# Bhasha-Open/Akshar

Hardware: NVIDIA B200
Metric: utf8_input_GBps_batch_encode (higher is better)
Workload: dtype u8

## Files before the change

akshar_b200/csrc/ak_abi_encode.inc:

```
extern "C" {

struct AkTokOut {
    void* ids;
    int64_t id_cap;
    int ids_u16;
    void* splits;
    int splits_i32;
};
static int ak_run_tok(akshar_ctx* ctx, AkCall& C, const AkBatch& B, int64_t max_bytes, int kind, const AkTokOut& O) {
    int rc;
    const AkTokWs W = ak_tok_ws(max_bytes, B.n_rows);
    char* base = C.ws + C.L.scratch;
    const size_t avail = C.ws_bytes - C.L.scratch;
    const size_t surplus = avail > W.total ? ((avail - W.total) / 4) & ~(size_t)255 : 0;
    const size_t pool_ints = W.pool_ints + surplus / 4, longpool_ints = W.longpool_ints + surplus / 4;
    char* longpool = base + W.longpool + surplus;
    char* sl = base + W.slots + 2 * surplus;
    const size_t left = avail - (W.slots + 2 * surplus) - 4096;
    const double per_wt = (double)left / ((double)W.n_wt * (AKT_SLOT_BYTES + 0.001));
    int cap = AKT_CAP_MIN, shift = 8;
    while (cap < AKT_CAP_MAX && (double)(2 * cap) <= per_wt) { cap *= 2; ++shift; }
    const size_t n_slots = (size_t)W.n_wt * (size_t)cap;
    AkSlots S;
    S.ev = (AkEvent*)sl;
    S.count = (uint32_t*)(base + W.count);
    S.cap = cap;
    S.shift = shift;
    unsigned long long* resolved = (unsigned long long*)(sl + ak_align(n_slots * 8));
    uint32_t* aux = (uint32_t*)(sl + 2 * ak_align(n_slots * 8));
    int32_t* wt_ids = (int32_t*)(base + W.wt_ids);
    int64_t* wt_base = (int64_t*)(base + W.wt_base);
    unsigned long long* wt_seg = (unsigned long long*)(base + W.wt_seg);
    float* wt_segx = (float*)(base + W.wt_segx);
    const size_t nscan = ak_align(((size_t)W.n_wt / AKS_TILE + 2) * 8);
    unsigned long long* scan_state0 = (unsigned long long*)(base + W.scan_state);
    unsigned long long* scan_state1 = (unsigned long long*)(base + W.scan_state + nscan);
    AkcTable& tc = ctx->tok_cache[kind];
    if (!ctx->wc_hold || tc.reset) {
        const unsigned long long limit = (1ull << tc.work.bits) / 4;
        ak_cache_guard_kernel<<<ctx->sm_count * 4, 256, 0, C.stream>>>(tc.work.e, tc.image, tc.bytes / 8, tc.work.inserted, limit, tc.reset ? 1 : 0);
        if ((rc = ak_after_launch(ctx, "tok-cache-guard"))) return rc;
        ak_cache_guard_reset_kernel<<<1, 1, 0, C.stream>>>(tc.work.inserted, limit, tc.reset ? 1 : 0);
        if ((rc = ak_after_launch(ctx, "tok-cache-guard-reset"))) return rc;
        tc.reset = false;
    }
    AK_CUDA(ctx, cudaMemsetAsync(base + W.row_flag, 0, ak_align((size_t)B.n_rows + 1), C.stream));
    AK_CUDA(ctx, cudaMemsetAsync(scan_state0, 0, 2 * nscan, C.stream));
    int* tickets = (int*)C.ws;
    unsigned int* any_flag = (unsigned int*)(C.ws + 144);
    unsigned long long* pool_used = (unsigned long long*)(C.ws + 152);
    const int64_t base0 = B.text_begin - (int64_t)(((uintptr_t)B.text + (uintptr_t)B.text_begin) & 15u);
    const int64_t span = (B.dyn_end ? max_bytes : B.text_end) - base0;
    const int64_t n_wt_ub = (span + AKT_WARP_BYTES) / AKT_WARP_BYTES;
    AkWordsArgs A;
    A.B = B;
    A.T = ctx->T;
    A.bpe = ctx->bpe_d;
    A.base0 = base0;
    A.wrow = (const int64_t*)(base + W.wrow);
    A.S = S;
    A.row_flag = (uint8_t*)(base + W.row_flag);
    A.any_flag = any_flag;
    A.row_ev = (uint32_t*)(base + W.row_ev);
    long long* n_wt_dev = (long long*)(C.ws + 136);
    A.n_wt_out = n_wt_dev;
    const int entries = (int)(n_wt_ub * 2 + 3);
    ak_warp_rows_kernel<<<(entries + 255) / 256, 256, 0, C.stream>>>(B, base0, entries, (int64_t*)(base + W.wrow));
    if ((rc = ak_after_launch(ctx, "tok-warp-rows"))) return rc;
    if (kind == 1) {
        ak_long_rows_kernel<<<ctx->sm_count * 4, 256, 0, C.stream>>>(B, AKT_LONG_ROW, A.row_flag, any_flag);
        if ((rc = ak_after_launch(ctx, "tok-long-rows"))) return rc;
    }
    {
        AkTimed tm(ctx, AKSHAR_TIMER_WORDS, C.stream);
        const int g = ak_grid(ctx, ctx->occ_words[kind], (int)((n_wt_ub + AKW_THREADS / 32 - 1) / (AKW_THREADS / 32)));
        if (kind == 0) ak_words_kernel<0><<<g, AKW_THREADS, 0, C.stream>>>(A);
        else ak_words_kernel<1><<<g, AKW_THREADS, 0, C.stream>>>(A);
    }
    if ((rc = ak_after_launch(ctx, "tok-words"))) return rc;
    AkLookupCtx X;
    X.M.kind = kind;
    X.M.bpe = ctx->bpe_d;
    X.M.uni = ctx->uni_d;
    X.M.cache = tc.work;
    X.M.pool.base = (int32_t*)longpool;
    X.M.pool.used = (unsigned long long*)(C.ws + 128);
    X.M.pool.cap = longpool_ints;
    X.M.T = ctx->T;
    X.text = nullptr;
    X.off = nullptr;
    X.n_rows = 0;
    X.tb = X.te = 0;
    X.result = nullptr;
    X.ids = O.ids;
    X.id_cap = O.id_cap;
    X.ids_u16 = O.ids_u16;
    X.splits = O.splits;
    X.splits_i32 = O.splits_i32;
    X.row_flag = A.row_flag;
    X.row_fix = (unsigned long long*)(base + W.row_fix);
    X.pool = (int32_t*)(base + W.pool);
    X.pool_used = pool_used;
    X.pool_cap = pool_ints;
    X.any_fix = 0;
    AkRowFixArgs R;
    R.B = B;
    R.X.M = X.M;
    R.X.text = nullptr;
    R.X.off = nullptr;
    R.X.n_rows = 0;
    R.X.result = nullptr;
    R.X.ev = S.ev;
    R.X.n_events = 0;
    R.X.row_ev = A.row_ev;
    R.X.row_fix = (unsigned long long*)(base + W.row_fix);
    R.X.pool = X.pool;
    R.X.pool_used = pool_used;
    R.X.pool_cap = pool_ints;
    R.base0 = base0;
    R.cap = cap;
    R.row_flag = A.row_flag;
    R.any_flag = any_flag;
    ak_rowfix_kernel<<<ctx->sm_count * 8, 128, 0, C.stream>>>(R);
    if ((rc = ak_after_launch(ctx, "tok-rowfix"))) return rc;
    const int warp_ctas = (int)((n_wt_ub + AKL_THREADS / 32 - 1) / (AKL_THREADS / 32));
    const int scan_tiles = (int)(n_wt_ub / AKS_TILE + 1);
    unsigned int* status_word = (unsigned int*)&B.result[2];
    AkResolveArgs Rs;
    Rs.B = B;
    Rs.X = X;
    Rs.base0 = base0;
    Rs.S = S;
    Rs.resolved = resolved;
    Rs.aux = aux;
    Rs.wt_ids = wt_ids;
    Rs.wt_seg = wt_seg;
    Rs.any_flag = any_flag;
    {
        AkTimed tm(ctx, kind == 0 ? AKSHAR_TIMER_BPE_ENCODE : AKSHAR_TIMER_UNIGRAM, C.stream);
        const int g = ak_grid(ctx, ctx->occ_resolve[kind], warp_ctas);
        if (kind == 0) ak_resolve_kernel<0><<<g, AKR_THREADS, 0, C.stream>>>(Rs);
        else ak_resolve_kernel<1><<<g, AKR_THREADS, 0, C.stream>>>(Rs);
    }
    if ((rc = ak_after_launch(ctx, "tok-resolve"))) return rc;
    if (kind == 1) {
        ak_scan_seg_kernel<<<ak_grid(ctx, 4, scan_tiles), AKS_THREADS, 0, C.stream>>>(wt_seg, n_wt_dev, wt_segx, tickets + 4, scan_state1, status_word);
        if ((rc = ak_after_launch(ctx, "tok-scan-seg"))) return rc;
        AkCheckArgs Ck;
        Ck.B = B;
        Ck.X = X;
        Ck.base0 = base0;
        Ck.S = S;
        Ck.resolved = resolved;
        Ck.aux = aux;
        Ck.wt_seg_before = wt_segx;
        Ck.wt_ids = wt_ids;
        Ck.any_flag = any_flag;
        ak_unicheck_kernel<<<ak_grid(ctx, ctx->occ_check, warp_ctas), AKL_THREADS, 0, C.stream>>>(Ck);
        if ((rc = ak_after_launch(ctx, "tok-check"))) return rc;
    }
    ak_scan_counts_kernel<<<ak_grid(ctx, 4, scan_tiles), AKS_THREADS, 0, C.stream>>>(wt_ids, 0, n_wt_dev, 1, wt_base, B.totals, tickets + 5, scan_state0,
                                                                                    status_word);
    if ((rc = ak_after_launch(ctx, "tok-scan-ids"))) return rc;
    AkEmitArgs E;
    E.B = B;
    E.X = X;
    E.base0 = base0;
    E.S = S;
    E.resolved = resolved;
    E.wt_base = wt_base;
    E.any_flag = any_flag;
    {
        AkTimed tm(ctx, AKSHAR_TIMER_EMIT, C.stream);
        if (O.ids_u16) ak_emit_kernel<uint16_t><<<ak_grid(ctx, ctx->occ_emit, warp_ctas), AKL_THREADS, 0, C.stream>>>(E);
        else ak_emit_kernel<int32_t><<<ak_grid(ctx, ctx->occ_emit, warp_ctas), AKL_THREADS, 0, C.stream>>>(E);
    }
    return ak_after_launch(ctx, "tok-emit");
}

static int ak_run_bpe(akshar_ctx* ctx, AkCall& C, const AkBatch& B, int64_t max_bytes, const AkTokOut& O) {
    return ak_run_tok(ctx, C, B, max_bytes, 0, O);
}

static int ak_run_unigram(akshar_ctx* ctx, AkCall& C, const AkBatch& B, int64_t max_bytes, const AkTokOut& O, int mode) {
    if (mode == AKSHAR_MODE_TILES && ctx->uni_fast) return ak_run_tok(ctx, C, B, max_bytes, 1, O);
    if (O.ids_u16 || O.splits_i32) {
        ctx->err = "compact outputs need AKSHAR_MODE_TILES and a model of the shape scripts/train_spm.py writes";
        return AKSHAR_E_ARG;
    }
    int32_t* d_ids = (int32_t*)O.ids;
    int64_t* d_id_splits = (int64_t*)O.splits;
    const int64_t id_capacity = O.id_cap;
    const size_t tiles = (size_t)ak_tiles_of(max_bytes, B.n_rows);
    AkUniArgs A;
    A.B = B;
    A.B.mode = AKSHAR_MODE_ROWS;
    A.B.n_tiles = (int)((B.n_rows + AK_ROWS_BLOCK - 1) / AK_ROWS_BLOCK);
    A.B.ticket = (int*)C.ws + 1;
    A.B.state0 = C.B.state0 + 1 * tiles;
    A.U = ctx->uni_d;
    A.back = (uint32_t*)(C.ws + C.L.scratch);
    A.back_cap = (int64_t)((C.ws_bytes - C.L.scratch) / 4);
    A.ids = d_ids;
    A.id_cap = id_capacity;
    A.id_splits = d_id_splits;
    {
        AkTimed tm(ctx, AKSHAR_TIMER_UNIGRAM, C.stream);
        ak_unigram_kernel<<<ak_grid(ctx, ctx->occ_uni, A.B.n_tiles), AK_ROWS_BLOCK, 0, C.stream>>>(A);
    }
    return ak_after_launch(ctx, "unigram");
}

int akshar_encode_bpe_batch(akshar_ctx* ctx, const uint8_t* d_text, const int64_t* d_row_offsets, int64_t n_rows,
                            int64_t text_begin, int64_t text_end, int mode, int32_t* d_ids, int64_t id_capacity,
                            int64_t* d_id_splits, int64_t* d_result, void* d_workspace, size_t workspace_bytes,
                            void* stream) {
    AkDeviceGuard device_guard(ctx ? ctx->device : 0);
    AkCall C;
    int rc = ak_begin(ctx, d_text, d_row_offsets, n_rows, text_begin, text_end, mode, 0, d_result, d_workspace, workspace_bytes,
                      stream, C);
    if (rc) return rc;
    if (!ctx->has_bpe) {
        ctx->err = "no BPE model loaded";
        return AKSHAR_E_NOMODEL;
    }
    if (!d_id_splits || id_capacity < 0 || (!d_ids && id_capacity > 0)) {
        ctx->err = "bad argument";
        return AKSHAR_E_ARG;
    }
    if (n_rows == 0) return ak_empty_rows(ctx, d_id_splits, nullptr, C.stream);
    const AkTokOut O = {d_ids, id_capacity, 0, d_id_splits, 0};
    return ak_run_bpe(ctx, C, C.B, text_end - text_begin, O);
}

int akshar_encode_unigram_batch(akshar_ctx* ctx, const uint8_t* d_text, const int64_t* d_row_offsets, int64_t n_rows,
                                int64_t text_begin, int64_t text_end, int mode, int32_t* d_ids, int64_t id_capacity,
                                int64_t* d_id_splits, int64_t* d_result, void* d_workspace, size_t workspace_bytes,
                                void* stream) {
    AkDeviceGuard device_guard(ctx ? ctx->device : 0);
    AkCall C;
    if (mode != AKSHAR_MODE_TILES && mode != AKSHAR_MODE_ROWS) return AKSHAR_E_ARG;
    int rc = ak_begin(ctx, d_text, d_row_offsets, n_rows, text_begin, text_end, AKSHAR_MODE_ROWS, AK_ROWS_BLOCK, d_result,
                      d_workspace, workspace_bytes, stream, C);
    if (rc) return rc;
    if (!ctx->has_uni) {
        ctx->err = "no Unigram model loaded";
        return AKSHAR_E_NOMODEL;
    }
    if (!d_id_splits || id_capacity < 0 || (!d_ids && id_capacity > 0)) {
        ctx->err = "bad argument";
        return AKSHAR_E_ARG;
    }
    if (n_rows == 0) return ak_empty_rows(ctx, d_id_splits, nullptr, C.stream);
    const AkTokOut O = {d_ids, id_capacity, 0, d_id_splits, 0};
    return ak_run_unigram(ctx, C, C.B, text_end - text_begin, O, mode);
}

int akshar_tokenizer_encode_batch(akshar_ctx* ctx, const uint8_t* d_text, const int64_t* d_row_offsets, int64_t n_rows,
                                  int64_t text_begin, int64_t text_end, uint32_t norm_flags, int kind, int mode,
                                  uint8_t* d_norm_text, int64_t norm_capacity, int64_t* d_norm_row_offsets, int32_t* d_ids,
                                  int64_t id_capacity, int64_t* d_id_splits, int64_t* d_result, void* d_workspace,
                                  size_t workspace_bytes, void* stream) {
    return akshar_tokenizer_encode_batch_ex(ctx, d_text, d_row_offsets, n_rows, text_begin, text_end, norm_flags, kind, mode,
                                            d_norm_text, norm_capacity, d_norm_row_offsets, d_ids, id_capacity, d_id_splits, 0u,
                                            d_result, d_workspace, workspace_bytes, stream);
}

int akshar_tokenizer_encode_batch_ex(akshar_ctx* ctx, const uint8_t* d_text, const int64_t* d_row_offsets, int64_t n_rows,
                                     int64_t text_begin, int64_t text_end, uint32_t norm_flags, int kind, int mode,
                                     uint8_t* d_norm_text, int64_t norm_capacity, int64_t* d_norm_row_offsets, void* d_ids,
                                     int64_t id_capacity, void* d_id_splits, uint32_t out_flags, int64_t* d_result,
                                     void* d_workspace, size_t workspace_bytes, void* stream) {
    AkDeviceGuard device_guard(ctx ? ctx->device : 0);
    if (!ctx) return AKSHAR_E_ARG;
    if (norm_capacity < 0 || !d_norm_row_offsets || (!d_norm_text && norm_capacity > 0) || (norm_flags & ~15u) ||
        (kind != 0 && kind != 1) || !d_id_splits || id_capacity < 0 || (!d_ids && id_capacity > 0) || (out_flags & ~3u)) {
        ctx->err = "bad argument";
        return AKSHAR_E_ARG;
    }
    if ((out_flags & AKSHAR_OUT_IDS_U16) && akshar_vocab_size(ctx, kind) > 65536) {
        ctx->err = "uint16 ids need a vocabulary of at most 65536 entries";
        return AKSHAR_E_ARG;
    }
    if (kind == 0 ? !ctx->has_bpe : !ctx->has_uni) {
        ctx->err = "no model loaded for this encoder";
        return AKSHAR_E_NOMODEL;
    }
    const int64_t n_bytes = text_end - text_begin;
    const int64_t max_bytes = n_bytes > norm_capacity ? n_bytes : norm_capacity;
    if (workspace_bytes < ak_ws_layout(max_bytes, n_rows).total) {
        ctx->err = "workspace too small: need " + std::to_string(ak_ws_layout(max_bytes, n_rows).total) + " bytes";
        return AKSHAR_E_WORKSPACE;
    }
    AkCall C;
    int rc = ak_begin(ctx, d_text, d_row_offsets, n_rows, text_begin, text_end, mode, 0, d_result, d_workspace, workspace_bytes,
                      stream, C);
    if (rc) return rc;
    C.L = ak_ws_layout(max_bytes, n_rows);
    const size_t tiles = (size_t)ak_tiles_of(max_bytes, n_rows);
    AK_CUDA(ctx, cudaMemsetAsync(C.ws, 0, 256 + ak_align(4 * tiles * 8), C.stream));
    C.B.state0 = (unsigned long long*)(C.ws + C.L.state);
    C.B.state1 = C.B.state0 + tiles;
    if (n_rows == 0) {
        AK_CUDA(ctx, cudaMemsetAsync(d_id_splits, 0, sizeof(int64_t), C.stream));
        return ak_empty_rows(ctx, d_norm_row_offsets, nullptr, C.stream);
    }
    AkBatch B1 = C.B;
    B1.totals = d_result + 1;
    if ((rc = ak_run_normalize(ctx, C, B1, norm_flags, d_norm_text, norm_capacity, d_norm_row_offsets))) return rc;
    AkBatch B2 = C.B;
    B2.text = d_norm_text;
    B2.off = d_norm_row_offsets;
    B2.text_begin = 0;
    B2.text_end = 0;
    B2.dyn_end = d_result + 1;
    if (mode != AKSHAR_MODE_TILES) B2.n_tiles = (int)((n_rows + AK_BLOCK - 1) / AK_BLOCK);
    const AkTokOut O = {d_ids, id_capacity, (out_flags & AKSHAR_OUT_IDS_U16) ? 1 : 0, d_id_splits, (out_flags & AKSHAR_OUT_SPLITS_I32) ? 1 : 0};
    if (kind == 0) return ak_run_bpe(ctx, C, B2, max_bytes, O);
    return ak_run_unigram(ctx, C, B2, max_bytes, O, mode);
}

}
```

akshar_b200/csrc/ak_abi_text.inc:

```
static int ak_run_normalize(akshar_ctx* ctx, AkCall& C, const AkBatch& B, uint32_t flags, uint8_t* out, int64_t out_cap,
                            int64_t* out_off) {
    const bool raw_fast = flags == AK_NORM_ROMAN;
    if ((flags == (AK_NORM_ROMAN | AK_NORM_CLEAN) || raw_fast) && B.mode == AKSHAR_MODE_TILES && !B.dyn_end) {
        AkFastNormArgs F;
        F.flags = flags;
        F.B = B;
        F.T = ctx->T;
        F.out = out;
        F.out_cap = out_cap;
        F.out_off = out_off;
        F.base0 = B.text_begin - (int64_t)(((uintptr_t)B.text + (uintptr_t)B.text_begin) & 15u);
        F.B.n_tiles = (int)((B.text_end - F.base0 + AKF_TILE) / AKF_TILE);
        int64_t* tile_row = (int64_t*)(C.ws + C.L.tile_row);
        F.tile_row = tile_row;
        const int entries = F.B.n_tiles * AKF_WARPS + 1;
        ak_warp_rows_kernel<<<(entries + 255) / 256, 256, 0, C.stream>>>(B, F.base0, entries, tile_row);
        int rc = ak_after_launch(ctx, "warp-rows");
        if (rc) return rc;
        AkNfWork W;
        const size_t nt = (size_t)F.B.n_tiles;
        char* wp = C.ws + C.L.scratch;
        W.info = (uint32_t*)wp;                         wp += ak_align(nt * AK_BLOCK * 4);
        W.tile_total = (int32_t*)wp;                    wp += ak_align(nt * AKF_WARPS * 4);
        W.tile_base = (int64_t*)wp;                     wp += ak_align((nt * AKF_WARPS + 1) * 8);
        W.slow = (AkSlowEntry*)wp;
        W.n_slow = (unsigned int*)(C.ws + 72);
        W.slow_cap = (unsigned int)(nt * AK_BLOCK / 16 + 1024);
        {
            AkTimed tm(ctx, AKSHAR_TIMER_NORMALIZE_CLASSIFY, C.stream);
            ak_nf3_classify_kernel<<<ak_grid(ctx, ctx->occ_nf3, F.B.n_tiles), AKN3_THREADS, 0, C.stream>>>(F, W);
        }
        if ((rc = ak_after_launch(ctx, "normalize-classify"))) return rc;
        AkNfSlowArgs S;
        S.B = B;
        S.T = ctx->T;
        S.W = W;
        S.tile_row = tile_row;
        S.out = out;
        S.out_cap = out_cap;
        S.out_off = out_off;
        S.write = 0;
        S.flags = flags;
        const int slow_grid = ctx->sm_count * AKN_SLOW_MINB;
        ak_nf_slow_kernel<<<slow_grid, 128, 0, C.stream>>>(S);
        if ((rc = ak_after_launch(ctx, "normalize-slow-count"))) return rc;
        const long long n_wtiles = (long long)F.B.n_tiles * AKF_WARPS;
        ak_scan_counts_kernel<<<ak_grid(ctx, 4, (int)(n_wtiles / AKS_TILE + 1)), AKS_THREADS, 0, C.stream>>>(
            W.tile_total, n_wtiles, nullptr, 1, W.tile_base, B.totals, (int*)C.ws + 6, C.B.state1,
            (unsigned int*)&B.result[2]);
        if ((rc = ak_after_launch(ctx, "normalize-scan"))) return rc;
        {
            AkTimed tm(ctx, AKSHAR_TIMER_NORMALIZE_WRITE, C.stream);
            ak_nf_write_kernel<<<ak_grid(ctx, ctx->occ_nf_write, F.B.n_tiles), AK_BLOCK, 0, C.stream>>>(F, W);
        }
        if ((rc = ak_after_launch(ctx, "normalize-write"))) return rc;
        S.write = 1;
        ak_nf_slow_kernel<<<slow_grid, 128, 0, C.stream>>>(S);
        return ak_after_launch(ctx, "normalize-slow-write");
    }
    AkNormArgs A;
    A.B = B;
    A.T = ctx->T;
    A.flags = flags;
    A.out = out;
    A.out_cap = out_cap;
    A.out_off = out_off;
    ak_normalize_kernel<<<ak_grid(ctx, ctx->occ_norm, A.B.n_tiles), AK_BLOCK, 0, C.stream>>>(A);
    return ak_after_launch(ctx, "normalize");
}

int akshar_normalize_batch(akshar_ctx* ctx, const uint8_t* d_text, const int64_t* d_row_offsets, int64_t n_rows,
                           int64_t text_begin, int64_t text_end, uint32_t flags, int mode, uint8_t* d_out_text,
                           int64_t out_capacity, int64_t* d_out_row_offsets, int64_t* d_result, void* d_workspace,
                           size_t workspace_bytes, void* stream) {
    AkDeviceGuard device_guard(ctx ? ctx->device : 0);
    AkCall C;
    int rc = ak_begin(ctx, d_text, d_row_offsets, n_rows, text_begin, text_end, mode, 0, d_result, d_workspace, workspace_bytes,
                      stream, C);
    if (rc) return rc;
    if (!d_out_row_offsets || out_capacity < 0 || (!d_out_text && out_capacity > 0) || (flags & ~15u)) {
        ctx->err = "bad argument";
        return AKSHAR_E_ARG;
    }
    if (n_rows == 0) return ak_empty_rows(ctx, d_out_row_offsets, nullptr, C.stream);
    return ak_run_normalize(ctx, C, C.B, flags, d_out_text, out_capacity, d_out_row_offsets);
}

static int ak_run_seg_mask(akshar_ctx* ctx, AkCall& C, const AkBatch& B, int64_t max_bytes, uint32_t flags, uint32_t* cmask,
                           uint32_t* rmask, uint32_t* tags, int64_t n_words) {
    int rc;
    AkSegMaskArgs M;
    M.B = B;
    M.T = ctx->T;
    M.flags = flags;
    M.shift = (int)(((uintptr_t)B.text + (uintptr_t)B.text_begin) & 15u);
    M.base0 = B.text_begin - M.shift;
    M.cmask = cmask;
    M.rmask = rmask;
    M.t0 = tags;
    M.t1 = tags ? tags + n_words : nullptr;
    M.n_words = n_words;
    const int64_t n_wt = (B.text_begin + max_bytes - M.base0 + AKN3_WARP_BYTES) / AKN3_WARP_BYTES;
    int64_t* wrow = (int64_t*)(C.ws + C.L.scratch);
    M.wrow = wrow;
    const int entries = (int)(n_wt * 2 + 3);
    ak_warp_rows_kernel<<<(entries + 255) / 256, 256, 0, C.stream>>>(B, M.base0, entries, wrow);
    if ((rc = ak_after_launch(ctx, "segment-warp-rows"))) return rc;
    {
        AkTimed tm(ctx, AKSHAR_TIMER_SEGMENT, C.stream);
        ak_seg_mask_kernel<<<ak_grid(ctx, 8, (int)((n_wt + AKSM_THREADS / 32 - 1) / (AKSM_THREADS / 32))), AKSM_THREADS, 0, C.stream>>>(M);
    }
    return ak_after_launch(ctx, "segment-mask");
}

int akshar_segment_batch(akshar_ctx* ctx, const uint8_t* d_text, const int64_t* d_row_offsets, int64_t n_rows,
                         int64_t text_begin, int64_t text_end, uint32_t flags, int mode, int32_t* d_cluster_ends,
                         int64_t cluster_capacity, int64_t* d_cluster_splits, int32_t* d_run_ends, uint8_t* d_run_tags,
                         int64_t run_capacity, int64_t* d_run_splits, int64_t* d_result, void* d_workspace,
                         size_t workspace_bytes, void* stream) {
    AkDeviceGuard device_guard(ctx ? ctx->device : 0);
    AkCall C;
    int rc = ak_begin(ctx, d_text, d_row_offsets, n_rows, text_begin, text_end, mode, 0, d_result, d_workspace, workspace_bytes,
                      stream, C);
    if (rc) return rc;
    const bool want_c = (flags & AKSHAR_SEG_CLUSTERS) != 0, want_r = (flags & AKSHAR_SEG_RUNS) != 0;
    if (flags & AKSHAR_SEG_MASK) {
        const int64_t n_words = (text_end - text_begin + 32) / 32;
        if ((flags & ~15u) || (!want_c && !want_r) || ((flags & AKSHAR_SEG_MATRAS) && !want_c) || mode != AKSHAR_MODE_TILES ||
            (want_c && (!d_cluster_ends || cluster_capacity < n_words)) ||
            (want_r && (!d_run_ends || !d_run_tags || run_capacity < n_words))) {
            ctx->err = "bad argument (AKSHAR_SEG_MASK: tile mode, capacities in 32-bit words >= (bytes + 32) / 32)";
            return AKSHAR_E_ARG;
        }
        return ak_run_seg_mask(ctx, C, C.B, text_end - text_begin, flags & 7u, (uint32_t*)d_cluster_ends, (uint32_t*)d_run_ends,
                               (uint32_t*)d_run_tags, n_words);
    }
    if ((flags & ~7u) || (!want_c && !want_r) || ((flags & AKSHAR_SEG_MATRAS) && !want_c) ||
        (want_c && (!d_cluster_splits || cluster_capacity < 0 || (!d_cluster_ends && cluster_capacity > 0))) ||
        (want_r && (!d_run_splits || run_capacity < 0 || ((!d_run_ends || !d_run_tags) && run_capacity > 0)))) {
        ctx->err = "bad argument";
        return AKSHAR_E_ARG;
    }
    if (n_rows == 0) return ak_empty_rows(ctx, want_c ? d_cluster_splits : nullptr, want_r ? d_run_splits : nullptr, C.stream);
    AkSegArgs A;
    A.B = C.B;
    A.T = ctx->T;
    A.flags = flags;
    A.o.cluster_ends = d_cluster_ends;
    A.o.cluster_splits = d_cluster_splits;
    A.o.run_ends = d_run_ends;
    A.o.run_tags = d_run_tags;
    A.o.run_splits = d_run_splits;
    A.o.cbase = A.o.rbase = 0;
    A.o.ccap = want_c ? cluster_capacity : 0;
    A.o.rcap = want_r ? run_capacity : 0;
    if (mode == AKSHAR_MODE_TILES) {
        AkSegOffArgs F;
        F.B = C.B;
        F.T = ctx->T;
        F.flags = flags;
        F.base0 = text_begin - (int64_t)(((uintptr_t)d_text + (uintptr_t)text_begin) & 15u);
        const int64_t n_wt = (text_end - F.base0 + AKN3_WARP_BYTES) / AKN3_WARP_BYTES;
        char* wp = C.ws + C.L.scratch;
        int64_t* wrow = (int64_t*)wp;       wp += ak_align(((size_t)n_wt * 2 + 3) * 8);
        F.c_count = (int32_t*)wp;           wp += ak_align((size_t)n_wt * 4);
        F.r_count = (int32_t*)wp;           wp += ak_align((size_t)n_wt * 4);
        int64_t* c_base = (int64_t*)wp;     wp += ak_align((size_t)n_wt * 8);
        int64_t* r_base = (int64_t*)wp;
        F.wrow = wrow;
        F.c_base = c_base;
        F.r_base = r_base;
        F.o = A.o;
        const int entries = (int)(n_wt * 2 + 3);
        ak_warp_rows_kernel<<<(entries + 255) / 256, 256, 0, C.stream>>>(C.B, F.base0, entries, wrow);
        if ((rc = ak_after_launch(ctx, "segment-warp-rows"))) return rc;
        const int grid = ak_grid(ctx, 8, (int)((n_wt + AKSO_THREADS / 32 - 1) / (AKSO_THREADS / 32)));
        ak_seg_off_kernel<false><<<grid, AKSO_THREADS, 0, C.stream>>>(F);
        if ((rc = ak_after_launch(ctx, "segment-count"))) return rc;
        const int sgrid = ak_grid(ctx, 4, (int)(n_wt / AKS_TILE + 1));
        if (want_c) {
            ak_scan_counts_kernel<<<sgrid, AKS_THREADS, 0, C.stream>>>(F.c_count, (long long)n_wt, nullptr, 1, c_base, d_result,
                                                                       (int*)C.ws + 5, C.B.state0, (unsigned int*)&d_result[2]);
            if ((rc = ak_after_launch(ctx, "segment-scan"))) return rc;
        }
        if (want_r) {
            ak_scan_counts_kernel<<<sgrid, AKS_THREADS, 0, C.stream>>>(F.r_count, (long long)n_wt, nullptr, 1, r_base, d_result + 1,
                                                                       (int*)C.ws + 6, C.B.state1, (unsigned int*)&d_result[2]);
            if ((rc = ak_after_launch(ctx, "segment-scan"))) return rc;
        }
        {
            AkTimed tm(ctx, AKSHAR_TIMER_SEGMENT, C.stream);
            ak_seg_off_kernel<true><<<grid, AKSO_THREADS, 0, C.stream>>>(F);
        }
        return ak_after_launch(ctx, "segment-emit");
    }
    ak_segment_kernel<<<ak_grid(ctx, ctx->occ_seg, A.B.n_tiles), AK_BLOCK, 0, C.stream>>>(A);
    return ak_after_launch(ctx, "segment");
}

int akshar_word_tokenize_batch(akshar_ctx* ctx, const uint8_t* d_text, const int64_t* d_row_offsets, int64_t n_rows,
                               int64_t text_begin, int64_t text_end, int rule, int32_t* d_word_begin, int32_t* d_word_end,
                               int64_t word_capacity, int64_t* d_word_splits, uint8_t* d_row_flags, int64_t* d_result,
                               void* d_workspace, size_t workspace_bytes, void* stream) {
    AkDeviceGuard device_guard(ctx ? ctx->device : 0);
    AkCall C;
    int rc = ak_begin(ctx, d_text, d_row_offsets, n_rows, text_begin, text_end, AKSHAR_MODE_TILES, 0, d_result, d_workspace,
                      workspace_bytes, stream, C);
    if (rc) return rc;
    if ((rule != AKSHAR_WORDS_HINDI && rule != AKSHAR_WORDS_SPLIT) || !d_word_splits || word_capacity < 0 ||
        ((!d_word_begin || !d_word_end) && word_capacity > 0)) {
        ctx->err = "bad argument";
        return AKSHAR_E_ARG;
    }
    if (n_rows == 0) return ak_empty_rows(ctx, d_word_splits, nullptr, C.stream);
    if (d_row_flags) AK_CUDA(ctx, cudaMemsetAsync(d_row_flags, 0, (size_t)n_rows, C.stream));
    AkWtArgs A;
    A.B = C.B;
    A.base0 = text_begin - (int64_t)(((uintptr_t)d_text + (uintptr_t)text_begin) & 15u);
    const int64_t n_wt = (text_end - A.base0 + AKT_WARP_BYTES) / AKT_WARP_BYTES;
    char* wp = C.ws + C.L.scratch;
    int64_t* wrow = (int64_t*)wp;       wp += ak_align(((size_t)n_wt * 2 + 3) * 8);
    A.count = (int32_t*)wp;             wp += ak_align((size_t)n_wt * 4);
    int64_t* wt_base = (int64_t*)wp;
    A.wrow = wrow;
    A.base = wt_base;
    A.mode = rule == AKSHAR_WORDS_HINDI ? AKW_MODE_HINDI : AKW_MODE_SPLIT;
    A.begin = d_word_begin;
    A.end = d_word_end;
    A.cap = word_capacity;
    A.splits = d_word_splits;
    A.row_flags = d_row_flags;
    const int entries = (int)(n_wt * 2 + 3);
    ak_warp_rows_kernel<<<(entries + 255) / 256, 256, 0, C.stream>>>(C.B, A.base0, entries, wrow);
    if ((rc = ak_after_launch(ctx, "words-warp-rows"))) return rc;
    const int grid = ak_grid(ctx, 8, (int)((n_wt + AKWT_THREADS / 32 - 1) / (AKWT_THREADS / 32)));
    ak_wtok_kernel<false><<<grid, AKWT_THREADS, 0, C.stream>>>(A);
    if ((rc = ak_after_launch(ctx, "words-count"))) return rc;
    ak_scan_counts_kernel<<<ak_grid(ctx, 4, (int)(n_wt / AKS_TILE + 1)), AKS_THREADS, 0, C.stream>>>(
        A.count, (long long)n_wt, nullptr, 1, wt_base, d_result, (int*)C.ws + 5, C.B.state0, (unsigned int*)&d_result[2]);
    if ((rc = ak_after_launch(ctx, "words-scan"))) return rc;
    {
        AkTimed tm(ctx, AKSHAR_TIMER_WORDTOK, C.stream);
        ak_wtok_kernel<true><<<grid, AKWT_THREADS, 0, C.stream>>>(A);
    }
    return ak_after_launch(ctx, "words-emit");
}
```

akshar_b200/csrc/ak_common.cuh:

```cuda
#pragma once
#define AK_BLOCK 256
#define AK_SPAN 32
#define AK_TILE (AK_BLOCK * AK_SPAN)
#define AK_LOOKBACK_LIMIT 4096
#define AK_ROWS_BLOCK 128
#define AKF_WARPS (AK_BLOCK / 32)
#define AKF_TILE (AKF_WARPS * AKF_WARP_BYTES)

static_assert((int)AK_ST_OVERFLOW == (int)AKSHAR_ST_OVERFLOW && (int)AK_ST_NFC_SEGMENT == (int)AKSHAR_ST_NFC_SEGMENT &&
              (int)AK_ST_PATHOLOGICAL == (int)AKSHAR_ST_PATHOLOGICAL && (int)AK_ST_ALPHABET == (int)AKSHAR_ST_ALPHABET &&
              (int)AK_ST_SPIN == (int)AKSHAR_ST_SPIN && (int)AK_ST_WORD == (int)AKSHAR_ST_WORD &&
              (int)AK_ST_INTERNAL == (int)AKSHAR_ST_INTERNAL && (int)AK_ST_BAD_ID == (int)AKSHAR_ST_BAD_ID, "status bits out of sync");
static_assert(AK_NORM_ROMAN == AKSHAR_NORM_ROMAN && AK_NORM_CLEAN == AKSHAR_NORM_CLEAN && AK_NORM_FILTER == AKSHAR_NORM_FILTER &&
              AK_NORM_COLLAPSE == AKSHAR_NORM_COLLAPSE && AK_NORM_NO_NFC == AKSHAR_NORM_NO_NFC, "flags out of sync");
static_assert(AK_SEG_CLUSTERS == AKSHAR_SEG_CLUSTERS && AK_SEG_MATRAS == AKSHAR_SEG_MATRAS &&
              AK_SEG_RUNS == AKSHAR_SEG_RUNS, "flags out of sync");

struct AkBatch {
    const uint8_t* text;
    const int64_t* off;
    int64_t n_rows, text_begin, text_end;
    int mode;
    int n_tiles;
    int* ticket;
    unsigned long long* state0;
    unsigned long long* state1;
    int64_t* result;
    int64_t* totals;
    const unsigned int* run_if;
    const int64_t* dyn_end;
};

__device__ __forceinline__ bool ak_batch_begin(AkBatch& B) {
    if (B.run_if && *B.run_if == 0) return false;
    if (B.dyn_end) {
        if (B.result[2] & (AK_ST_OVERFLOW | AK_ST_PATHOLOGICAL | AK_ST_NFC_SEGMENT | AK_ST_SPIN)) return false;
        B.text_end = B.text_begin + *B.dyn_end;
        if (B.mode == AKSHAR_MODE_TILES) B.n_tiles = (int)((B.text_end - B.text_begin + AK_TILE) / AK_TILE);
    }
    return true;
}

struct AkSpan {
    int64_t s, e, r_lo, r_hi, limit;
};

__device__ __forceinline__ void ak_raise(int64_t* result, uint32_t bits) {
    if (bits) atomicOr((unsigned long long*)&result[2], (unsigned long long)bits);
}

__device__ __forceinline__ AkSpan ak_span_of(const AkBatch& B, int tile, int64_t* sh) {
    AkSpan sp;
    if (B.mode == AKSHAR_MODE_TILES) {
        const int64_t t0 = B.text_begin + (int64_t)tile * AK_TILE;
        int64_t t1 = t0 + AK_TILE;
        if (t1 > B.text_end + 1) t1 = B.text_end + 1;
        if (threadIdx.x == 0) {
            int64_t lo = ak_row_lower_bound(B.off, 0, B.n_rows, t0);
            sh[0] = lo > 0 ? lo - 1 : 0;
            sh[1] = ak_row_lower_bound(B.off, lo, B.n_rows, t1);
        }
        __syncthreads();
        sp.r_lo = sh[0];
        sp.r_hi = sh[1];
        sp.s = t0 + (int64_t)threadIdx.x * AK_SPAN;
        sp.e = sp.s + AK_SPAN;
        if (sp.e > t1) sp.e = t1;
        if (sp.s > sp.e) sp.s = sp.e;
        sp.limit = AK_LOOKBACK_LIMIT;
    } else {
        const int64_t r = (int64_t)tile * AK_BLOCK + threadIdx.x;
        sp.r_lo = 0;
        sp.r_hi = B.n_rows;
        sp.limit = 0;
        if (r < B.n_rows) {
            sp.s = B.off[r];
            sp.e = (r == B.n_rows - 1) ? B.text_end + 1 : B.off[r + 1];
        } else {
            sp.s = sp.e = 0;
        }
    }
    return sp;
}

__device__ __forceinline__ int ak_next_tile(int* ticket, int* sh) {
    __syncthreads();
    if (threadIdx.x == 0) *sh = atomicAdd(ticket, 1);
    __syncthreads();
    return *sh;
}



__global__ void ak_warp_rows_kernel(AkBatch B, int64_t base0, int n_entries, int64_t* wrow) {
    if (!ak_batch_begin(B)) return;
    const int k = blockIdx.x * blockDim.x + threadIdx.x;
    if (k >= n_entries) return;
    const int64_t pos = base0 + (int64_t)k * AKF_WARP_BYTES;
    int64_t r = ak_row_lower_bound(B.off, 0, B.n_rows, pos);
    if (B.off[r] < pos) r = B.n_rows + 1;
    wrow[k] = r;
}


#define AKN3_THREADS 128
#define AKN3_WARP_BYTES 960

__device__ __forceinline__ uint32_t akn3_lane_rows(const int64_t* off, int64_t n_rows, int64_t r_w0, int64_t ws, int lane) {
    uint32_t rows = 0;
    const int64_t lo = ws - 32, hi = ws + AKN3_WARP_BYTES + 32;
    for (int64_t r = r_w0;; r += 32) {
        const int64_t mr = r + lane;
        const int64_t p = mr <= n_rows ? off[mr] : hi;
        const unsigned m = __ballot_sync(0xFFFFFFFFu, p < hi);
        const int cnt = __popc(m);
        for (int j = 0; j < cnt; ++j) {
            const int rel = (int)(__shfl_sync(0xFFFFFFFFu, p, j) - lo);
            if ((rel >> 5) == lane) rows |= 1u << (rel & 31);
        }
        if (cnt < 32) break;
    }
    for (int64_t r = r_w0 - 1;; r -= 32) {
        const int64_t mr = r - lane;
        const int64_t p = mr >= 0 ? off[mr] : lo - 1;
        const unsigned m = __ballot_sync(0xFFFFFFFFu, p >= lo);
        const int cnt = __popc(m);
        for (int j = 0; j < cnt; ++j) {
            const int rel = (int)(__shfl_sync(0xFFFFFFFFu, p, j) - lo);
            if ((rel >> 5) == lane) rows |= 1u << (rel & 31);
        }
        if (cnt < 32) break;
    }
    return rows;
}

__device__ __forceinline__ uint32_t akn3_lane_rows2(const int64_t* off, int64_t n_rows, int64_t r_w0, int64_t ws, int lane,
                                                    int64_t& first_row, int& nrows) {
    uint32_t rows = 0;
    int64_t first = 0x7FFFFFFFFFFFFFFFll;
    int cntl = 0;
    const int64_t lo = ws - 32, hi = ws + AKN3_WARP_BYTES + 32;
    for (int64_t r = r_w0;; r += 32) {
        const int64_t mr = r + lane;
        const int64_t p = mr <= n_rows ? off[mr] : hi;
        const unsigned m = __ballot_sync(0xFFFFFFFFu, p < hi);
        const int cnt = __popc(m);
        for (int j = 0; j < cnt; ++j) {
            const int rel = (int)(__shfl_sync(0xFFFFFFFFu, p, j) - lo);
            if ((rel >> 5) == lane) {
                rows |= 1u << (rel & 31);
                ++cntl;
                if (r + j < first) first = r + j;
            }
        }
        if (cnt < 32) break;
    }
    for (int64_t r = r_w0 - 1;; r -= 32) {
        const int64_t mr = r - lane;
        const int64_t p = mr >= 0 ? off[mr] : lo - 1;
        const unsigned m = __ballot_sync(0xFFFFFFFFu, p >= lo);
        const int cnt = __popc(m);
        for (int j = 0; j < cnt; ++j) {
            const int rel = (int)(__shfl_sync(0xFFFFFFFFu, p, j) - lo);
            if ((rel >> 5) == lane) {
                rows |= 1u << (rel & 31);
                ++cntl;
                if (r - j < first) first = r - j;
            }
        }
        if (cnt < 32) break;
    }
    first_row = first;
    nrows = cntl;
    return rows;
}

__device__ __forceinline__ void akn3_load_edge(const uint8_t* text, int64_t cs, int lo, int hi, uint32_t* x) {
#pragma unroll
    for (int w = 0; w < 8; ++w) {
        uint32_t v = 0;
#pragma unroll
        for (int b = 0; b < 4; ++b) {
            const int i = 4 * w + b;
            if (i >= lo && i < hi) v |= (uint32_t)text[cs + i] << (8 * b);
        }
        x[w] = v;
    }
}
```

akshar_b200/csrc/ak_kernels.cu:

```cuda
#include <cuda_runtime.h>
#include <math.h>
#include <stdio.h>
#include <stdlib.h>
#include <string.h>

#include <exception>
#include <new>
#include <string>
#include <vector>

#include "../../include/akshar_b200.h"
#include "ak_models.h"
#include "ak_scan.cuh"
#include "ak_subword.cuh"
#include "ak_fast.cuh"
#include "ak_norm3.cuh"
#include "ak_seg3.cuh"
#include "ak_bpe3.cuh"
#include "ak_tok.cuh"
#include "ak_tok_host.h"
#include "ak_decode_host.h"
#include "unicode_tables.inc"


#include "ak_common.cuh"
#include "ak_norm_kernels.cuh"
#include "ak_seg_kernels.cuh"
#include "ak_sub_kernels.cuh"
#include "ak_tok_kernels.cuh"
#include "ak_wtok_kernels.cuh"
#include "ak_decode_kernels.cuh"
#include "ak_feat_kernels.cuh"
#include "ak_lines_kernels.cuh"

struct AkcTable {
    AkWordCache work{};
    unsigned long long* image = nullptr;
    size_t bytes = 0;
    bool reset = false;
};

struct akshar_ctx {
    int device = 0;
    int sm_count = 148;
    AkTables T{};
    std::vector<void*> allocs;
    std::string err;
    int64_t launches = 0;
    bool has_bpe = false, has_uni = false;
    AkBpeHost bpe_h;
    AkBpeDev bpe_d{};
    AkUniHost uni_h;
    AkUniDev uni_d{};
    std::vector<void*> bpe_allocs, uni_allocs;
    AkcTable tok_cache[2];
    AkDecTable dec[2][2] = {};
    bool uni_fast = false;
    int occ_words[2] = {0, 0}, occ_resolve[2] = {0, 0}, occ_check = 0, occ_emit = 0;
    bool timing = false;
    bool wc_hold = false;
    cudaEvent_t tev[AKSHAR_TIMER_COUNT][2] = {};
    bool tev_valid[AKSHAR_TIMER_COUNT] = {};
    int occ_norm = 0, occ_seg = 0, occ_uni = 0, occ_sig = 0, occ_nf_write = 0, occ_nf3 = 0;
};

struct AkDeviceGuard {
    int prev = -1;
    bool switched = false;
    explicit AkDeviceGuard(int dev) {
        if (cudaGetDevice(&prev) == cudaSuccess && prev != dev) switched = cudaSetDevice(dev) == cudaSuccess;
    }
    ~AkDeviceGuard() {
        if (switched) cudaSetDevice(prev);
    }
};

#define AK_CUDA(ctx, call)                                                                         \
    do {                                                                                           \
        cudaError_t e_ = (call);                                                                   \
        if (e_ != cudaSuccess) {                                                                   \
            (ctx)->err = std::string(#call) + ": " + cudaGetErrorString(e_);                       \
            return AKSHAR_E_CUDA;                                                                  \
        }                                                                                          \
    } while (0)

template <class V>
static int ak_upload(akshar_ctx* ctx, std::vector<void*>& owner, const V* src, size_t n, const V** dst) {
    void* d = nullptr;
    size_t bytes = (n ? n : 1) * sizeof(V);
    AK_CUDA(ctx, cudaMalloc(&d, bytes));
    owner.push_back(d);
    if (n) AK_CUDA(ctx, cudaMemcpy(d, src, n * sizeof(V), cudaMemcpyHostToDevice));
    *dst = (const V*)d;
    return 0;
}

extern "C" {

int akshar_version(void) { return 100; }

const char* akshar_status_str(int code) {
    switch (code) {
        case AKSHAR_OK: return "ok";
        case AKSHAR_E_ARG: return "bad argument";
        case AKSHAR_E_CUDA: return "CUDA error";
        case AKSHAR_E_MODEL: return "model could not be parsed or uses an unsupported configuration";
        case AKSHAR_E_NOMODEL: return "no model loaded for this encoder";
        case AKSHAR_E_WORKSPACE: return "workspace too small";
        default: return "unknown";
    }
}

int akshar_ctx_create(int device, akshar_ctx** out) {
    if (!out) return AKSHAR_E_ARG;
    *out = nullptr;
    akshar_ctx* ctx = new (std::nothrow) akshar_ctx();
    if (!ctx) return AKSHAR_E_ARG;
    ctx->device = device;
    *out = ctx;
    AkDeviceGuard device_guard(device);
    AK_CUDA(ctx, cudaSetDevice(device));
    cudaDeviceProp prop;
    AK_CUDA(ctx, cudaGetDeviceProperties(&prop, device));
    if (prop.major < 10) {
        ctx->err = "akshar_b200 is built for sm_100a (B200); device is sm_" + std::to_string(prop.major * 10 + prop.minor);
        return AKSHAR_E_CUDA;
    }
    ctx->sm_count = prop.multiProcessorCount;
    int rc;
#define UP(field, arr, n, type) \
    if ((rc = ak_upload<type>(ctx, ctx->allocs, (const type*)(arr), (size_t)(n), (const type**)&ctx->T.field))) return rc;
    UP(page_index, ak_tbl_page_index, AK_N_PAGES, uint16_t)
    UP(leaves, ak_tbl_leaves, AK_N_LEAF_PAGES * 256, uint32_t)
    UP(decomp_keys, ak_tbl_decomp_keys, AK_N_DECOMP, uint32_t)
    UP(decomp_off, ak_tbl_decomp_off, AK_N_DECOMP + 1, uint16_t)
    UP(decomp_data, ak_tbl_decomp_data, AK_N_DECOMP_DATA, uint32_t)
    UP(pair_keys, ak_tbl_pair_keys, AK_N_PAIRS, unsigned long long)
    UP(pair_vals, ak_tbl_pair_vals, AK_N_PAIRS, uint32_t)
    UP(ll_keys, ak_tbl_latin_lower_keys, AK_N_LATIN_LOWER, uint32_t)
    UP(ll_vals, ak_tbl_latin_lower_vals, AK_N_LATIN_LOWER, uint32_t)
    UP(fl_keys, ak_tbl_full_lower_keys, AK_N_FULL_LOWER, uint32_t)
    UP(fl_vals, ak_tbl_full_lower_vals, AK_N_FULL_LOWER, uint32_t)
    UP(kmap_keys, ak_tbl_kmap_keys, AK_N_KMAP, uint32_t)
    UP(kmap_off, ak_tbl_kmap_off, AK_N_KMAP + 1, uint16_t)
    UP(kmap_data, ak_tbl_kmap_data, AK_N_KMAP_DATA, uint32_t)
    UP(hf_unknown, ak_tbl_hf_unknown, AK_N_HF_UNKNOWN, uint32_t)
#undef UP
    ctx->T.n_decomp = AK_N_DECOMP;
    ctx->T.n_pairs = AK_N_PAIRS;
    ctx->T.n_ll = AK_N_LATIN_LOWER;
    ctx->T.n_fl = AK_N_FULL_LOWER;
    ctx->T.n_kmap = AK_N_KMAP;
    ctx->T.n_hf_unknown = AK_N_HF_UNKNOWN;
    AK_CUDA(ctx, cudaOccupancyMaxActiveBlocksPerMultiprocessor(&ctx->occ_norm, ak_normalize_kernel, AK_BLOCK, 0));
    AK_CUDA(ctx, cudaOccupancyMaxActiveBlocksPerMultiprocessor(&ctx->occ_nf_write, ak_nf_write_kernel, AK_BLOCK, 0));
    AK_CUDA(ctx, cudaOccupancyMaxActiveBlocksPerMultiprocessor(&ctx->occ_nf3, ak_nf3_classify_kernel, AKN3_THREADS, 0));
    AK_CUDA(ctx, cudaOccupancyMaxActiveBlocksPerMultiprocessor(&ctx->occ_seg, ak_segment_kernel, AK_BLOCK, 0));
    AK_CUDA(ctx, cudaOccupancyMaxActiveBlocksPerMultiprocessor(&ctx->occ_uni, ak_unigram_kernel, AK_ROWS_BLOCK, 0));
    AK_CUDA(ctx, cudaOccupancyMaxActiveBlocksPerMultiprocessor(&ctx->occ_sig, ak_signature_kernel, AK_ROWS_BLOCK, 0));
    AK_CUDA(ctx, cudaOccupancyMaxActiveBlocksPerMultiprocessor(&ctx->occ_words[0], ak_words_kernel<0>, AKW_THREADS, 0));
    AK_CUDA(ctx, cudaOccupancyMaxActiveBlocksPerMultiprocessor(&ctx->occ_words[1], ak_words_kernel<1>, AKW_THREADS, 0));
    AK_CUDA(ctx, cudaOccupancyMaxActiveBlocksPerMultiprocessor(&ctx->occ_resolve[0], ak_resolve_kernel<0>, AKR_THREADS, 0));
    AK_CUDA(ctx, cudaOccupancyMaxActiveBlocksPerMultiprocessor(&ctx->occ_resolve[1], ak_resolve_kernel<1>, AKR_THREADS, 0));
    AK_CUDA(ctx, cudaOccupancyMaxActiveBlocksPerMultiprocessor(&ctx->occ_check, ak_unicheck_kernel, AKL_THREADS, 0));
    AK_CUDA(ctx, cudaOccupancyMaxActiveBlocksPerMultiprocessor(&ctx->occ_emit, ak_emit_kernel<int32_t>, AKL_THREADS, 0));
    return AKSHAR_OK;
}

static void ak_free_list(std::vector<void*>& v) {
    for (void* p : v) cudaFree(p);
    v.clear();
}

void akshar_ctx_destroy(akshar_ctx* ctx) {
    if (!ctx) return;
    AkDeviceGuard device_guard(ctx->device);
    ak_free_list(ctx->allocs);
    ak_free_list(ctx->bpe_allocs);
    ak_free_list(ctx->uni_allocs);
    for (int i = 0; i < AKSHAR_TIMER_COUNT; ++i)
        for (int k = 0; k < 2; ++k)
            if (ctx->tev[i][k]) cudaEventDestroy(ctx->tev[i][k]);
    delete ctx;
}

const char* akshar_last_error(akshar_ctx* ctx) { return ctx ? ctx->err.c_str() : "null context"; }

int akshar_word_cache_hold(akshar_ctx* ctx, int hold) {
    if (!ctx) return AKSHAR_E_ARG;
    if (hold < 0) {
        ctx->tok_cache[0].reset = ctx->tok_cache[1].reset = true;
        return AKSHAR_OK;
    }
    ctx->wc_hold = hold != 0;
    return AKSHAR_OK;
}

int akshar_timing_enable(akshar_ctx* ctx, int enable) {
    AkDeviceGuard device_guard(ctx ? ctx->device : 0);
    if (!ctx) return AKSHAR_E_ARG;
    AK_CUDA(ctx, cudaSetDevice(ctx->device));
    if (enable)
        for (int i = 0; i < AKSHAR_TIMER_COUNT; ++i)
            for (int k = 0; k < 2; ++k)
                if (!ctx->tev[i][k]) AK_CUDA(ctx, cudaEventCreate(&ctx->tev[i][k]));
    ctx->timing = enable != 0;
    for (int i = 0; i < AKSHAR_TIMER_COUNT; ++i) ctx->tev_valid[i] = false;
    return AKSHAR_OK;
}

int akshar_timing_read(akshar_ctx* ctx, int timer, float* ms) {
    if (!ctx || !ms || timer < 0 || timer >= AKSHAR_TIMER_COUNT) return AKSHAR_E_ARG;
    if (!ctx->tev_valid[timer]) return AKSHAR_E_ARG;
    AK_CUDA(ctx, cudaEventSynchronize(ctx->tev[timer][1]));
    AK_CUDA(ctx, cudaEventElapsedTime(ms, ctx->tev[timer][0], ctx->tev[timer][1]));
    return AKSHAR_OK;
}

int64_t akshar_launch_count(akshar_ctx* ctx) { return ctx ? ctx->launches : 0; }

static inline size_t ak_align(size_t x) { return (x + 255) & ~(size_t)255; }
static inline int64_t ak_tiles_of(int64_t n_bytes, int64_t n_rows) {
    int64_t a = (n_bytes + n_bytes / 8 + 1024 + 32 + AKF_TILE - 1) / AKF_TILE;
    int64_t b = (n_rows + AK_ROWS_BLOCK - 1) / AK_ROWS_BLOCK;
    return (a > b ? a : b) + 1;
}
struct AkTokWs {
    size_t wrow, count, wt_ids, wt_base, wt_seg, wt_segx, scan_state, row_flag, row_ev, row_fix, pool, longpool, slots, total;
    size_t pool_ints, longpool_ints;
    int64_t n_wt;
};
#define AKT_CAP_MIN 256
#define AKT_CAP_MAX 2048
#define AKT_SLOT_BYTES 20
static AkTokWs ak_tok_ws(int64_t n_bytes, int64_t n_rows) {
    AkTokWs W;
    W.n_wt = n_bytes / AKT_WARP_BYTES + 3;
    size_t at = 0;
    W.wrow = at;       at += ak_align(((size_t)W.n_wt * 2 + 4) * 8);
    W.count = at;      at += ak_align((size_t)W.n_wt * 4);
    W.wt_ids = at;     at += ak_align((size_t)W.n_wt * 4);
    W.wt_base = at;    at += ak_align((size_t)W.n_wt * 8);
    W.wt_seg = at;     at += ak_align((size_t)W.n_wt * 8);
    W.wt_segx = at;    at += ak_align((size_t)W.n_wt * 4);
    W.scan_state = at; at += 2 * ak_align(((size_t)W.n_wt / AKS_TILE + 2) * 8);
    W.row_flag = at;   at += ak_align((size_t)n_rows + 1);
    W.row_ev = at;     at += ak_align(((size_t)n_rows + 2) * 4);
    W.row_fix = at;    at += ak_align(((size_t)n_rows + 1) * 8);
    W.pool_ints = (size_t)n_bytes / 4 + 65536;
    W.pool = at;       at += ak_align(W.pool_ints * 4);
    W.longpool_ints = (size_t)n_bytes / 8 + 65536;
    W.longpool = at;   at += ak_align(W.longpool_ints * 4);
    W.slots = at;
    at += (size_t)W.n_wt * AKT_CAP_MIN * (AKT_SLOT_BYTES + 1) + 8192;
    W.total = at;
    return W;
}

struct AkWsLayout {
    size_t control, state, tile_row, scratch, total;
};
static AkWsLayout ak_ws_layout(int64_t n_bytes, int64_t n_rows) {
    AkWsLayout L;
    size_t tiles = (size_t)ak_tiles_of(n_bytes, n_rows);
    L.control = 0;
    L.state = 256;
    L.tile_row = L.state + ak_align(4 * tiles * 8);
    size_t at = L.tile_row + ak_align(8 * (tiles * AKF_WARPS + 2));
    L.scratch = at;
    size_t m = 4 * (size_t)(n_bytes + 2 * n_rows + 2);
    const size_t nf = ak_align(tiles * AK_BLOCK * 4) + ak_align(tiles * AKF_WARPS * 4) + ak_align((tiles * AKF_WARPS + 1) * 8) +
                      ak_align((tiles * AK_BLOCK / 16 + 1024) * sizeof(AkSlowEntry));
    if (nf > m) m = nf;
    const size_t n_wt = (size_t)n_bytes / AKN3_WARP_BYTES + 3;
    const size_t sg = ak_align((2 * n_wt + 3) * 8) + 2 * ak_align(n_wt * 4) + 2 * ak_align(n_wt * 8);
    if (sg > m) m = sg;
    const size_t tok = ak_tok_ws(n_bytes, n_rows).total;
    if (tok > m) m = tok;
    L.total = at + ak_align(m);
    return L;
}

size_t akshar_workspace_bytes(int64_t n_bytes, int64_t n_rows) {
    if (n_bytes < 0 || n_rows < 0) return 0;
    return ak_ws_layout(n_bytes, n_rows).total;
}

struct AkCall {
    akshar_ctx* ctx;
    AkBatch B;
    AkWsLayout L;
    char* ws;
    size_t ws_bytes;
    cudaStream_t stream;
};

static int ak_begin(akshar_ctx* ctx, const uint8_t* d_text, const int64_t* d_row_offsets, int64_t n_rows, int64_t text_begin,
                    int64_t text_end, int mode, int rows_block, int64_t* d_result, void* d_workspace, size_t workspace_bytes,
                    void* stream, AkCall& C) {
    if (!ctx) return AKSHAR_E_ARG;
    if (!d_row_offsets || !d_result || n_rows < 0 || text_end < text_begin || (!d_text && text_end > text_begin) ||
        (mode != AKSHAR_MODE_TILES && mode != AKSHAR_MODE_ROWS)) {
        ctx->err = "bad argument";
        return AKSHAR_E_ARG;
    }
    const int64_t n_bytes = text_end - text_begin;
    if (n_bytes >= AKSHAR_MAX_CALL_BYTES || n_rows >= AKSHAR_MAX_CALL_ROWS) {
        ctx->err = "batch too large for one call: at most 4 GiB - 64 KiB of text and 2^29 - 1 rows; split it by row ranges";
        return AKSHAR_E_ARG;
    }
    C.ctx = ctx;
    C.L = ak_ws_layout(n_bytes, n_rows);
    if (!d_workspace || workspace_bytes < C.L.total) {
        ctx->err = "workspace too small: need " + std::to_string(C.L.total) + " bytes";
        return AKSHAR_E_WORKSPACE;
    }
    C.ws = (char*)d_workspace;
    C.ws_bytes = workspace_bytes;
    C.stream = (cudaStream_t)stream;
    AK_CUDA(ctx, cudaSetDevice(ctx->device));
    const size_t tiles = (size_t)ak_tiles_of(n_bytes, n_rows);
    AK_CUDA(ctx, cudaMemsetAsync(C.ws, 0, 256 + ak_align(4 * tiles * 8), C.stream));
    AK_CUDA(ctx, cudaMemsetAsync(d_result, 0, 4 * sizeof(int64_t), C.stream));
    AkBatch& B = C.B;
    B.text = d_text;
    B.off = d_row_offsets;
    B.n_rows = n_rows;
    B.text_begin = text_begin;
    B.text_end = text_end;
    B.mode = mode;
    if (rows_block > 0) B.n_tiles = (int)((n_rows + rows_block - 1) / rows_block);
    else if (mode == AKSHAR_MODE_TILES) B.n_tiles = (int)((n_bytes + 1 + AK_TILE - 1) / AK_TILE);
    else B.n_tiles = (int)((n_rows + AK_BLOCK - 1) / AK_BLOCK);
    B.ticket = (int*)C.ws;
    B.state0 = (unsigned long long*)(C.ws + C.L.state);
    B.state1 = B.state0 + tiles;
    B.result = d_result;
    B.totals = d_result;
    B.run_if = nullptr;
    B.dyn_end = nullptr;
    return AKSHAR_OK;
}

struct AkTimed {
    akshar_ctx* ctx;
    int slot;
    cudaStream_t s;
    AkTimed(akshar_ctx* c, int sl, cudaStream_t st) : ctx(c), slot(sl), s(st) {
        if (ctx->timing && ctx->tev[slot][0]) cudaEventRecord(ctx->tev[slot][0], s);
    }
    ~AkTimed() {
        if (ctx->timing && ctx->tev[slot][1]) { cudaEventRecord(ctx->tev[slot][1], s); ctx->tev_valid[slot] = true; }
    }
};

static int ak_grid(akshar_ctx* ctx, int occ, int n_tiles) {
    int g = ctx->sm_count * (occ > 0 ? occ : 1);
    return n_tiles < g ? (n_tiles > 0 ? n_tiles : 1) : g;
}

static int ak_after_launch(akshar_ctx* ctx, const char* what) {
    cudaError_t e = cudaGetLastError();
    static const bool debug_sync = getenv("AKSHAR_DEBUG_SYNC") != nullptr;
    if (e == cudaSuccess && debug_sync) {
        e = cudaDeviceSynchronize();
        if (e != cudaSuccess) fprintf(stderr, "akshar_b200: kernel '%s' failed: %s\n", what, cudaGetErrorString(e));
    }
    if (e != cudaSuccess) {
        ctx->err = std::string(what) + " launch: " + cudaGetErrorString(e);
        return AKSHAR_E_CUDA;
    }
    ctx->launches++;
    return AKSHAR_OK;
}

static int ak_empty_rows(akshar_ctx* ctx, int64_t* a, int64_t* b, cudaStream_t s) {
    if (a) AK_CUDA(ctx, cudaMemsetAsync(a, 0, sizeof(int64_t), s));
    if (b) AK_CUDA(ctx, cudaMemsetAsync(b, 0, sizeof(int64_t), s));
    return AKSHAR_OK;
}

#include "ak_abi_text.inc"

}

#include "ak_abi_aux.inc"
#include "ak_abi_models.inc"
#include "ak_abi_encode.inc"
```

akshar_b200/csrc/ak_norm_kernels.cuh:

```cuda
#pragma once
struct AkNormArgs {
    AkBatch B;
    AkTables T;
    uint32_t flags;
    uint8_t* out;
    int64_t out_cap;
    int64_t* out_off;
};

__global__ void __launch_bounds__(AK_BLOCK) ak_normalize_kernel(const AkNormArgs A) {
    __shared__ int ws[33];
    __shared__ int s_tile;
    __shared__ int64_t s_win[2];
    __shared__ long long s_base;
    AkBatch B = A.B;
    if (!ak_batch_begin(B)) return;
    for (;;) {
        const int tile = ak_next_tile(B.ticket, &s_tile);
        if (tile >= B.n_tiles) break;
        const AkSpan sp = ak_span_of(B, tile, s_win);
        uint32_t st = 0;
        int cnt = 0;
        if (sp.s < sp.e)
            cnt = (int)ak_norm_span(A.T, B.text, B.off, B.n_rows, sp.r_lo, sp.r_hi, sp.s, sp.e, A.flags, sp.limit, nullptr,
                                    nullptr, 0, st);
        int total;
        const int pre = ak_block_exscan<AK_BLOCK>(cnt, ws, total);
        if (threadIdx.x < 32) {
            long long b = ak_tile_prefix(B.state0, tile, total, (unsigned int*)&B.result[2], AK_ST_SPIN);
            if (threadIdx.x == 0) {
                s_base = b;
                if (tile == B.n_tiles - 1) B.totals[0] = b + total;
            }
        }
        __syncthreads();
        const int64_t obase = s_base + pre;
        if (sp.s < sp.e) {
            uint8_t* o = nullptr;
            if (obase + cnt <= A.out_cap) o = A.out + obase;
            else if (cnt > 0) st |= AK_ST_OVERFLOW;
            uint32_t st2 = 0;
            ak_norm_span(A.T, B.text, B.off, B.n_rows, sp.r_lo, sp.r_hi, sp.s, sp.e, A.flags, sp.limit, o, A.out_off, obase, st2);
        }
        ak_raise(B.result, st);
    }
}

struct AkFastNormArgs {
    AkBatch B;
    AkTables T;
    uint8_t* out;
    int64_t out_cap;
    int64_t* out_off;
    const int64_t* tile_row;
    int64_t base0;
    uint32_t flags;
};

__device__ __noinline__ void akf_load_edge(const uint8_t* text, int64_t cs, int lo, int hi, uint32_t* w) {
    w[0] = w[1] = w[2] = w[3] = 0;
#pragma unroll 1
    for (int i = lo; i < hi; ++i) w[i >> 2] |= (uint32_t)text[cs + i] << ((i & 3) * 8);
}

template <class CH>
__device__ __forceinline__ void akf_load_chunk(const uint8_t* text, int64_t cs, int64_t tb, int64_t te, CH& c) {
    int64_t lo = tb - cs, hi = te - cs;
    lo = lo < 0 ? 0 : (lo > 16 ? 16 : lo);
    hi = hi < 0 ? 0 : (hi > 16 ? 16 : hi);
    c.own = hi > lo ? (((1u << hi) - 1u) & ~((1u << lo) - 1u)) : 0u;
    if (c.own == 0xFFFFu) {
        const uint4 v = *reinterpret_cast<const uint4*>(text + cs);
        c.w[0] = v.x; c.w[1] = v.y; c.w[2] = v.z; c.w[3] = v.w;
    } else {
        uint32_t w[4];
        akf_load_edge(text, cs, (int)lo, (int)hi, w);
        c.w[0] = w[0]; c.w[1] = w[1]; c.w[2] = w[2]; c.w[3] = w[3];
    }
}


#define AK_SLOW_BYTES 72
struct AkSlowEntry {
    int64_t pos;
    int64_t out_base;
    int32_t cnt;
    int32_t tile;
    int32_t span;
    int32_t pad_;
    uint8_t bytes[AK_SLOW_BYTES];
};

struct AkNfWork {
    uint32_t* info;
    int32_t* tile_total;
    int64_t* tile_base;
    AkSlowEntry* slow;
    unsigned int* n_slow;
    unsigned int slow_cap;
};

template <class CH>
__device__ __forceinline__ void akf_load_lane(const AkBatch& B, int64_t cs, CH& c) {
    akf_load_chunk(B.text, cs, B.text_begin, B.text_end, c);
    uint32_t nx = __shfl_down_sync(0xFFFFFFFFu, c.w[0], 1);
    if ((threadIdx.x & 31) == 31) {
        nx = 0;
#pragma unroll
        for (int i = 0; i < 4; ++i) {
            const int64_t q = cs + 16 + i;
            if (q >= B.text_begin && q < B.text_end) nx |= (uint32_t)B.text[q] << (i * 8);
        }
    }
    c.w[4] = nx;
}


#ifndef AKN3_MINB
#define AKN3_MINB 8
#endif
__global__ void __launch_bounds__(AKN3_THREADS, AKN3_MINB) ak_nf3_classify_kernel(const AkFastNormArgs A, const AkNfWork W) {
    const AkBatch& B = A.B;
    const int tid = threadIdx.x, lane = tid & 31, warp = tid >> 5;
    const int64_t tb = B.text_begin, te = B.text_end;
    const bool raw = !(A.flags & AK_NORM_CLEAN);
    for (int tile = blockIdx.x; tile < B.n_tiles; tile += gridDim.x) {
        const int64_t tile_start = A.base0 + (int64_t)tile * AKF_TILE;
        const int64_t ws = tile_start + (int64_t)warp * AKN3_WARP_BYTES;
        const int64_t cs = ws + (int64_t)(lane - 1) * 32;
        AkN3Lane L;
        {
            uint32_t x[8];
            int64_t lo = tb - cs, hi = te - cs;
            lo = lo < 0 ? 0 : (lo > 32 ? 32 : lo);
            hi = hi < 0 ? 0 : (hi > 32 ? 32 : hi);
            if (lo == 0 && hi == 32) {
                const uint4 v0 = *reinterpret_cast<const uint4*>(B.text + cs);
                const uint4 v1 = *reinterpret_cast<const uint4*>(B.text + cs + 16);
                x[0] = v0.x; x[1] = v0.y; x[2] = v0.z; x[3] = v0.w;
                x[4] = v1.x; x[5] = v1.y; x[6] = v1.z; x[7] = v1.w;
                L.own = 0xFFFFFFFFu;
            } else {
                akn3_load_edge(B.text, cs, (int)lo, (int)hi, x);
                L.own = hi > lo ? ((hi == 32 ? 0xFFFFFFFFu : ((1u << hi) - 1u)) & ~((1u << lo) - 1u)) : 0u;
            }
            L.rows = akn3_lane_rows(B.off, B.n_rows, A.tile_row[(size_t)tile * AKF_WARPS + 2 * warp], ws, lane);
            akn3_phase1(x, L);
        }
        uint32_t up1p = __shfl_up_sync(0xFFFFFFFFu, L.up1, 1);
        uint32_t dn1n = __shfl_down_sync(0xFFFFFFFFu, L.dn1, 1);
        if (lane == 0) up1p = 0;
        if (lane == 31) dn1n = 0;
        akn3_phase2(L, up1p, dn1n, raw);
        uint32_t up2p = __shfl_up_sync(0xFFFFFFFFu, L.up2, 1);
        uint32_t dn2n = __shfl_down_sync(0xFFFFFFFFu, L.dn2, 1);
        if (lane == 0) up2p = AKN3_HALO_UP2;
        if (lane == 31) dn2n = 0;
        akn3_phase3(A.T, B.text, cs, te, L, up2p, dn2n, raw);
        {
            uint32_t rest = 0;
            if (L.ge) rest = akn3_gaps_local(B.text, cs, te, L);
            if (lane == 0) {
                akn3_gaps_remote(B.text, cs, te, L, rest, 0u);
                rest = 0;
            }
            if (__any_sync(0xFFFFFFFFu, rest != 0u)) {
                const uint32_t lk = akn3_last_kept(B.text, cs, te, L);
                const uint32_t plk = __shfl_up_sync(0xFFFFFFFFu, lk, 1);
                akn3_gaps_remote(B.text, cs, te, L, rest, plk);
            }
        }
        akn3_phase3b(L);
        const uint32_t up3p = __shfl_up_sync(0xFFFFFFFFu, L.up3, 1);
        const uint32_t dn3n = __shfl_down_sync(0xFFFFFFFFu, L.dn3, 1);
        uint32_t info[2] = {0u, 0u};
        const bool fast = akn3_phase4(L, up3p, dn1n, dn3n, info[0], info[1]);
        int cnt = 0;
        if (lane >= 1 && lane <= 30) {
            bool act[2];
#pragma unroll
            for (int h = 0; h < 2; ++h) {
                const int64_t hs = cs + 16 * h;
                const int64_t ss = hs < tb ? tb : hs;
                const int64_t se = hs + 16 > te + 1 ? te + 1 : hs + 16;
                act[h] = ss < se;
            }
            uint32_t v[2] = {0u, 0u};
            if (fast) {
                if (act[0]) { v[0] = info[0]; cnt += __popc(v[0]); }
                if (act[1]) { v[1] = info[1]; cnt += __popc(v[1]); }
            } else if (act[0] || act[1]) {
                const unsigned int idx = atomicAdd(W.n_slow, 1u);
                if (idx < W.slow_cap) {
                    AkSlowEntry e;
                    e.pos = act[0] ? cs : cs + 16;
                    e.out_base = 0;
                    e.cnt = 0;
                    e.tile = tile * AKF_WARPS + 2 * warp + (lane >> 4);
                    e.span = (act[0] && act[1]) ? 32 : 16;
                    e.pad_ = 0;
                    W.slow[idx] = e;
                } else {
                    ak_raise(B.result, AK_ST_PATHOLOGICAL);
                }
                if (act[0]) { v[0] = 0x80000000u | idx; if (act[1]) v[1] = 0xC0000000u | idx; }
                else v[1] = 0x80000000u | idx;
            }
#pragma unroll
            for (int h = 0; h < 2; ++h) {
                const int k = (int)((cs + 16 * h - tile_start) >> 4);
                W.info[(size_t)tile * AK_BLOCK + (k / AKF_REAL) * 32 + 1 + (k % AKF_REAL)] = v[h];
            }
        }
        if (tid < 2 * AKF_WARPS) W.info[(size_t)tile * AK_BLOCK + (tid >> 1) * 32 + (tid & 1) * 31] = 0;
#pragma unroll
        for (int d = 8; d > 0; d >>= 1) cnt += __shfl_xor_sync(0xFFFFFFFFu, cnt, d);
        if ((lane & 15) == 0) W.tile_total[(size_t)tile * AKF_WARPS + 2 * warp + (lane >> 4)] = cnt;
    }
}

struct AkNfSlowArgs {
    AkBatch B;
    AkTables T;
    AkNfWork W;
    const int64_t* tile_row;
    uint8_t* out;
    int64_t out_cap;
    int64_t* out_off;
    int write;
    uint32_t flags;
};

#ifndef AKN_SLOW_MINB
#define AKN_SLOW_MINB 12
#endif
__global__ void __launch_bounds__(128, AKN_SLOW_MINB) ak_nf_slow_kernel(const AkNfSlowArgs A) {
    const AkBatch& B = A.B;
    unsigned int n = *A.W.n_slow;
    if (n > A.W.slow_cap) n = A.W.slow_cap;
    const uint32_t NFLAGS = A.flags;
    for (unsigned int j = blockIdx.x * blockDim.x + threadIdx.x; j < n; j += gridDim.x * blockDim.x) {
        AkSlowEntry e = A.W.slow[j];
        const int64_t ss = e.pos < B.text_begin ? B.text_begin : e.pos;
        const int64_t se = e.pos + e.span > B.text_end + 1 ? B.text_end + 1 : e.pos + e.span;
        const size_t cta_tile = (size_t)e.tile / AKF_WARPS;
        const int64_t r0 = A.tile_row[cta_tile * AKF_WARPS], r1 = A.tile_row[(cta_tile + 1) * AKF_WARPS];
        const int64_t rlo = r0 > 0 ? r0 - 1 : 0, rhi = r1 > B.n_rows ? B.n_rows : r1;
        uint32_t st = 0;
        if (!A.write) {
            const int cnt = (int)ak_norm_span(A.T, B.text, B.off, B.n_rows, rlo, rhi, ss, se, NFLAGS, AK_LOOKBACK_LIMIT,
                                              A.W.slow[j].bytes, A.out_off, 0, st, AK_SLOW_BYTES);
            A.W.slow[j].cnt = cnt;
            atomicAdd(&A.W.tile_total[e.tile], cnt);
        } else if (e.cnt > AK_SLOW_BYTES) {
            uint8_t* dst = (e.out_base + e.cnt <= A.out_cap) ? A.out + e.out_base : nullptr;
            ak_norm_span(A.T, B.text, B.off, B.n_rows, rlo, rhi, ss, se, NFLAGS, AK_LOOKBACK_LIMIT, dst, A.out_off, e.out_base, st);
        }
        ak_raise(B.result, st);
    }
}

__device__ __forceinline__ void akf_write_run(const AkChunk& c, uint32_t emit, uint8_t* dst) {
    uint32_t w[7];
#pragma unroll
    for (int j = 0; j < 5; ++j) {
        const uint32_t x = c.w[j];
        const uint32_t t7 = x & 0x7F7F7F7Fu;
        const uint32_t up = ((t7 + 0x3F3F3F3Fu) & ~(t7 + 0x25252525u) & ~x) & 0x80808080u;
        w[j] = x | (up >> 2);
    }
    w[5] = w[6] = 0;
    const int a = __ffs(emit) - 1, n = __popc(emit);
    int h = (int)((4u - ((uint32_t)(uintptr_t)dst & 3u)) & 3u);
    if (h > n) h = n;
    const int t = a + h;
    const uint32_t sh = (uint32_t)(t & 3) * 8u;
    uint32_t x[6];
#pragma unroll
    for (int j = 0; j < 6; ++j) x[j] = t >= 4 ? w[j + 1] : w[j];
    uint32_t f[5];
#pragma unroll
    for (int j = 0; j < 5; ++j) f[j] = __funnelshift_r(x[j], x[j + 1], sh);
    {
        const uint32_t hv = __funnelshift_r(w[0], w[1], (uint32_t)a * 8u);
        if (h > 0) dst[0] = (uint8_t)hv;
        if (h > 1) dst[1] = (uint8_t)(hv >> 8);
        if (h > 2) dst[2] = (uint8_t)(hv >> 16);
    }
    const int nw = (n - h) >> 2, r = (n - h) & 3;
    uint32_t* d32 = reinterpret_cast<uint32_t*>(dst + h);
#pragma unroll
    for (int m = 0; m < 4; ++m) if (m < nw) d32[m] = f[m];
    const uint32_t tv = nw == 0 ? f[0] : nw == 1 ? f[1] : nw == 2 ? f[2] : nw == 3 ? f[3] : f[4];
    uint8_t* dt = dst + h + 4 * nw;
    if (r > 0) dt[0] = (uint8_t)tv;
    if (r > 1) dt[1] = (uint8_t)(tv >> 8);
    if (r > 2) dt[2] = (uint8_t)(tv >> 16);
}

#define AKF_WSTAGE (AKF_WARP_BYTES + 160)
__global__ void __launch_bounds__(AK_BLOCK) ak_nf_write_kernel(const AkFastNormArgs A, const AkNfWork W) {
    __shared__ __align__(16) uint8_t stage_all[AKF_WARPS][AKF_WSTAGE + 32];
    const AkBatch& B = A.B;
    const int lane = threadIdx.x & 31, warp = threadIdx.x >> 5;
    uint8_t* stage = stage_all[warp];
    const long long n_wt = (long long)B.n_tiles * AKF_WARPS;
    for (long long wt = (long long)blockIdx.x * AKF_WARPS + warp; wt < n_wt; wt += (long long)gridDim.x * AKF_WARPS) {
        const int64_t ws0 = A.base0 + wt * AKF_WARP_BYTES;
        const int64_t r0 = A.tile_row[wt], r1 = A.tile_row[wt + 1];
        const int64_t cs = ws0 + (int64_t)(lane - 1) * 16;
        AkChunk c;
        akf_load_lane(B, cs, c);
        const uint32_t info = W.info[(size_t)wt * 32 + lane];
        const bool slow = (info & 0x80000000u) != 0;
        const bool cont = slow && (info & 0x40000000u);
        const unsigned int sidx = info & 0x3FFFFFFFu;
        int cnt = 0;
        if (slow) { if (sidx < W.slow_cap && !cont) cnt = W.slow[sidx].cnt; }
        else cnt = __popc(info);
        int inc = cnt;
#pragma unroll
        for (int d = 1; d < 32; d <<= 1) {
            const int y = __shfl_up_sync(0xFFFFFFFFu, inc, d);
            if (lane >= d) inc += y;
        }
        const int total = __shfl_sync(0xFFFFFFFFu, inc, 31);
        const int pre = inc - cnt;
        const int64_t base = W.tile_base[wt];
        const bool fits = base + total <= A.out_cap;
        const bool staged = fits && total <= AKF_WSTAGE;
        const int pad = (int)((uintptr_t)(A.out + base) & 15);
        if (!fits && lane == 0 && total > 0) ak_raise(B.result, AK_ST_OVERFLOW);
        if (slow) {
            if (sidx < W.slow_cap && !cont) {
                W.slow[sidx].out_base = base + pre;
                if (cnt <= AK_SLOW_BYTES && fits) {
                    uint8_t* dst = staged ? stage + pad + pre : A.out + base + pre;
                    const uint8_t* src = W.slow[sidx].bytes;
                    for (int i = 0; i < cnt; ++i) dst[i] = src[i];
                }
            }
        } else if (info && fits) {
            uint8_t* dst = staged ? stage + pad + pre : A.out + base + pre;
            const uint32_t lowbit = info & (0u - info);
            if (staged && ((info + lowbit) & info) == 0u && lowbit <= 8u) akf_write_run(c, info, dst);
            else akf_write(c, info, dst);
        }
        __syncwarp();
        if (staged) {
            uint8_t* g = A.out + base;
            int head = (16 - pad) & 15;
            if (head > total) head = total;
            if (lane < head) g[lane] = stage[pad + lane];
            const int body = (total - head) >> 4;
            for (int i = lane; i < body; i += 32)
                *reinterpret_cast<uint4*>(g + head + 16 * i) = *reinterpret_cast<const uint4*>(stage + pad + head + 16 * i);
            const int tail0 = head + (body << 4);
            if (lane < total - tail0) g[tail0 + lane] = stage[pad + tail0 + lane];
        }
        const int64_t r_end = r1 <= B.n_rows ? r1 : B.n_rows + 1;
        for (int64_t rr = r0; rr < r_end; rr += 32) {
            const int64_t r = rr + lane;
            const bool have = r < r_end;
            const int rel = have ? (int)(B.off[r] - ws0) : 0;
            const int th = 1 + (rel >> 4), i = rel & 15;
            const uint32_t e = __shfl_sync(0xFFFFFFFFu, info, th);
            const int p = __shfl_sync(0xFFFFFFFFu, pre, th);
            if (!have) continue;
            if (!(e & 0x80000000u)) A.out_off[r] = base + p + __popc(e & ((1u << i) - 1u));
            else {
                int64_t adj = 0;
                if ((e & 0x40000000u) && (e & 0x3FFFFFFFu) < W.slow_cap) adj = W.slow[e & 0x3FFFFFFFu].cnt;
                A.out_off[r] += base + p - adj;
            }
        }
        __syncwarp();
    }
}
```

akshar_b200/csrc/ak_seg_kernels.cuh:

```cuda
#pragma once
struct AkSegArgs {
    AkBatch B;
    AkTables T;
    uint32_t flags;
    AkSegOut o;
};

__global__ void __launch_bounds__(AK_BLOCK) ak_segment_kernel(const AkSegArgs A) {
    __shared__ int ws[33];
    __shared__ int s_tile;
    __shared__ int64_t s_win[2];
    __shared__ long long s_base[2];
    AkBatch B = A.B;
    if (!ak_batch_begin(B)) return;
    for (;;) {
        const int tile = ak_next_tile(B.ticket, &s_tile);
        if (tile >= B.n_tiles) break;
        const AkSpan sp = ak_span_of(B, tile, s_win);
        uint32_t st = 0;
        int64_t cc = 0, rc = 0;
        AkSegOut o = A.o;
        if (sp.s < sp.e)
            ak_seg_span(A.T, B.text, B.off, B.n_rows, sp.r_lo, sp.r_hi, sp.s, sp.e, A.flags, sp.limit, false, o, cc, rc, st);
        int ctot, rtot;
        const int cpre = ak_block_exscan<AK_BLOCK>((int)cc, ws, ctot);
        const int rpre = ak_block_exscan<AK_BLOCK>((int)rc, ws, rtot);
        if (threadIdx.x < 32) {
            long long cb = ak_tile_prefix(B.state0, tile, ctot, (unsigned int*)&B.result[2], AK_ST_SPIN);
            long long rb = ak_tile_prefix(B.state1, tile, rtot, (unsigned int*)&B.result[2], AK_ST_SPIN);
            if (threadIdx.x == 0) {
                s_base[0] = cb;
                s_base[1] = rb;
                if (tile == B.n_tiles - 1) { B.totals[0] = cb + ctot; B.totals[1] = rb + rtot; }
            }
        }
        __syncthreads();
        if (sp.s < sp.e) {
            o.cbase = s_base[0] + cpre;
            o.rbase = s_base[1] + rpre;
            if (o.cbase + cc > o.ccap || o.rbase + rc > o.rcap) st |= AK_ST_OVERFLOW;
            uint32_t st2 = 0;
            int64_t c2, r2;
            ak_seg_span(A.T, B.text, B.off, B.n_rows, sp.r_lo, sp.r_hi, sp.s, sp.e, A.flags, sp.limit, true, o, c2, r2, st2);
        }
        ak_raise(B.result, st);
    }
}


struct AkSegOffArgs {
    AkBatch B;
    AkTables T;
    uint32_t flags;
    const int64_t* wrow;
    int64_t base0;
    int32_t* c_count;
    int32_t* r_count;
    const int64_t* c_base;
    const int64_t* r_base;
    AkSegOut o;
};

#define AKSO_THREADS 128
template <bool EMIT>
__global__ void __launch_bounds__(AKSO_THREADS, 8) ak_seg_off_kernel(const AkSegOffArgs A) {
    AkBatch B = A.B;
    if (!ak_batch_begin(B)) return;
    const bool want_c = (A.flags & AK_SEG_CLUSTERS) != 0, want_r = (A.flags & AK_SEG_RUNS) != 0;
    const bool matras = (A.flags & AK_SEG_MATRAS) != 0;
    const int lane = threadIdx.x & 31, warp = threadIdx.x >> 5;
    const int64_t tb = B.text_begin, te = B.text_end;
    const long long n_wt = (te - A.base0 + AKN3_WARP_BYTES) / AKN3_WARP_BYTES;
    uint32_t st = 0;
    for (long long wt = (long long)blockIdx.x * (AKSO_THREADS / 32) + warp; wt < n_wt; wt += (long long)gridDim.x * (AKSO_THREADS / 32)) {
        const int64_t ws = A.base0 + wt * AKN3_WARP_BYTES;
        const int64_t r_w0 = A.wrow[2 * wt], r_w2 = A.wrow[2 * wt + 2];
        const int64_t cs = ws + (int64_t)(lane - 1) * 32;
        AkS3Lane L;
        {
            uint32_t x[8];
            int64_t lo = tb - cs, hi = te - cs;
            lo = lo < 0 ? 0 : (lo > 32 ? 32 : lo);
            hi = hi < 0 ? 0 : (hi > 32 ? 32 : hi);
            if (lo == 0 && hi == 32) {
                const uint4 v0 = *reinterpret_cast<const uint4*>(B.text + cs);
                const uint4 v1 = *reinterpret_cast<const uint4*>(B.text + cs + 16);
                x[0] = v0.x; x[1] = v0.y; x[2] = v0.z; x[3] = v0.w;
                x[4] = v1.x; x[5] = v1.y; x[6] = v1.z; x[7] = v1.w;
                L.own = 0xFFFFFFFFu;
            } else {
                akn3_load_edge(B.text, cs, (int)lo, (int)hi, x);
                L.own = hi > lo ? ((hi == 32 ? 0xFFFFFFFFu : ((1u << hi) - 1u)) & ~((1u << lo) - 1u)) : 0u;
            }
            L.rows = akn3_lane_rows(B.off, B.n_rows, r_w0, ws, lane);
            aks3_phase1(x, L);
        }
        uint32_t dn1n = __shfl_down_sync(0xFFFFFFFFu, L.dn1, 1);
        if (lane == 31) dn1n = 0;
        aks3_phase2(L, dn1n);
        if (L.FOR) aks3_foreign(A.T, B.text, cs, te, L);
        aks3_summary(L);
        const uint32_t up2p = __shfl_up_sync(0xFFFFFFFFu, L.up2, 1);
        const bool real = lane >= 1 && lane <= 30;
        const int64_t ss = cs < tb ? tb : cs;
        const int64_t se = cs + 32 > te + 1 ? te + 1 : cs + 32;
        const bool active = real && ss < se;
        int64_t nr = 0;
        if (EMIT) {
            const int mine = real ? __popc(L.rows) : 0;
            int inc = mine;
#pragma unroll
            for (int d = 1; d < 32; d <<= 1) {
                const int y = __shfl_up_sync(0xFFFFFFFFu, inc, d);
                if (lane >= d) inc += y;
            }
            nr = r_w0 + (inc - mine);
            if (active) while (nr <= B.n_rows && B.off[nr] < ss) ++nr;
        }
        const uint32_t tb_bit = (tb >= cs && tb < cs + 32) ? 1u << (int)(tb - cs) : 0u;
        const uint32_t rows_ev = L.rows & ~tb_bit;
        const int64_t rlo = r_w0 > 0 ? r_w0 - 1 : 0, rhi = r_w2 > B.n_rows ? B.n_rows : r_w2;
        bool slow = false;
        int cc = 0, rc = 0;
        if (active) {
            slow = !aks3_phase3(L, up2p, tb_bit, matras, want_c, want_r);
            if (slow) {
                AkSegOut o = A.o;
                int64_t scc = 0, src = 0;
                ak_seg_span(A.T, B.text, B.off, B.n_rows, rlo, rhi, ss, se, A.flags, AK_LOOKBACK_LIMIT, false, o, scc, src, st);
                cc = (int)scc;
                rc = (int)src;
            } else {
                const int nre = __popc(rows_ev);
                if (want_c) cc = __popc(L.brk) + nre;
                if (want_r) rc = __popc(L.rchg) + nre;
            }
        }
        int inc2 = cc | (rc << 16);
        const int mine2 = inc2;
#pragma unroll
        for (int d = 1; d < 32; d <<= 1) {
            const int y = __shfl_up_sync(0xFFFFFFFFu, inc2, d);
            if (lane >= d) inc2 += y;
        }
        if (!EMIT) {
            if (lane == 31) {
                A.c_count[wt] = inc2 & 0xFFFF;
                A.r_count[wt] = inc2 >> 16;
            }
            continue;
        }
        if (!active) continue;
        const int64_t cat = (want_c ? A.c_base[wt] : 0) + ((inc2 - mine2) & 0xFFFF);
        const int64_t rat = (want_r ? A.r_base[wt] : 0) + ((inc2 - mine2) >> 16);
        const bool fits = cat + cc <= A.o.ccap && rat + rc <= A.o.rcap;
        if (!fits) st |= AK_ST_OVERFLOW;
        if (slow) {
            AkSegOut o = A.o;
            o.cbase = cat;
            o.rbase = rat;
            if (!fits) o.ccap = o.rcap = 0;
            uint32_t st2 = 0;
            int64_t a, b;
            ak_seg_span(A.T, B.text, B.off, B.n_rows, rlo, rhi, ss, se, A.flags, AK_LOOKBACK_LIMIT, true, o, a, b, st2);
        } else {
            const uint32_t mc = want_c ? (L.brk | rows_ev) : 0u, mr = want_r ? (L.rchg | rows_ev) : 0u;
            if (fits) {
                const int64_t rs_in = nr > 0 ? B.off[nr - 1] : B.off[0];
                if (want_c) aks3_emit(L, mc, cs, rs_in, A.o.cluster_ends + cat, nullptr);
                if (want_r) aks3_emit(L, mr, cs, rs_in, A.o.run_ends + rat, A.o.run_tags + rat);
            }
            if (L.rows)
                aks3_splits(L, mc, mr, cs, B.off, B.n_rows, nr, cat, rat, want_c ? A.o.cluster_splits : nullptr,
                            want_r ? A.o.run_splits : nullptr);
        }
    }
    ak_raise(B.result, st);
}

struct AkSegMaskArgs {
    AkBatch B;
    AkTables T;
    uint32_t flags;
    const int64_t* wrow;
    int64_t base0;
    uint32_t* cmask;
    uint32_t* rmask;
    uint32_t* t0;
    uint32_t* t1;
    int64_t n_words;
    int shift;
};

#define AKSM_THREADS 128
#ifndef AKSM_MINB
#define AKSM_MINB 8
#endif
__global__ void __launch_bounds__(AKSM_THREADS, AKSM_MINB) ak_seg_mask_kernel(const AkSegMaskArgs A) {
    AkBatch B = A.B;
    if (!ak_batch_begin(B)) return;
    const bool want_c = (A.flags & AK_SEG_CLUSTERS) != 0, want_r = (A.flags & AK_SEG_RUNS) != 0;
    const bool matras = (A.flags & AK_SEG_MATRAS) != 0;
    const int lane = threadIdx.x & 31, warp = threadIdx.x >> 5;
    const int64_t tb = B.text_begin, te = B.text_end;
    const long long n_wt = (te - A.base0 + AKN3_WARP_BYTES) / AKN3_WARP_BYTES;
    uint32_t st = 0;
    long long n_c = 0, n_r = 0;
    for (long long wt = (long long)blockIdx.x * (AKSM_THREADS / 32) + warp; wt < n_wt; wt += (long long)gridDim.x * (AKSM_THREADS / 32)) {
        const int64_t ws = A.base0 + wt * AKN3_WARP_BYTES;
        const int64_t r_w0 = A.wrow[2 * wt], r_w2 = A.wrow[2 * wt + 2];
        const int64_t cs = ws + (int64_t)(lane - 1) * 32;
        AkS3Lane L;
        {
            uint32_t x[8];
            int64_t lo = tb - cs, hi = te - cs;
            lo = lo < 0 ? 0 : (lo > 32 ? 32 : lo);
            hi = hi < 0 ? 0 : (hi > 32 ? 32 : hi);
            if (lo == 0 && hi == 32) {
                const uint4 v0 = *reinterpret_cast<const uint4*>(B.text + cs);
                const uint4 v1 = *reinterpret_cast<const uint4*>(B.text + cs + 16);
                x[0] = v0.x; x[1] = v0.y; x[2] = v0.z; x[3] = v0.w;
                x[4] = v1.x; x[5] = v1.y; x[6] = v1.z; x[7] = v1.w;
                L.own = 0xFFFFFFFFu;
            } else {
                akn3_load_edge(B.text, cs, (int)lo, (int)hi, x);
                L.own = hi > lo ? ((hi == 32 ? 0xFFFFFFFFu : ((1u << hi) - 1u)) & ~((1u << lo) - 1u)) : 0u;
            }
            L.rows = akn3_lane_rows(B.off, B.n_rows, r_w0, ws, lane);
            aks3_phase1(x, L);
        }
        uint32_t dn1n = __shfl_down_sync(0xFFFFFFFFu, L.dn1, 1);
        if (lane == 31) dn1n = 0;
        aks3_phase2(L, dn1n);
        if (L.FOR) aks3_foreign(A.T, B.text, cs, te, L);
        aks3_summary(L);
        const uint32_t up2p = __shfl_up_sync(0xFFFFFFFFu, L.up2, 1);
        const int64_t ss = cs < tb ? tb : cs;
        const int64_t se = cs + 32 > te + 1 ? te + 1 : cs + 32;
        const bool active = lane >= 1 && ss < se;
        const uint32_t tb_bit = (tb >= cs && tb < cs + 32) ? 1u << (int)(tb - cs) : 0u;
        uint32_t mc = 0, mr = 0, t0 = 0, t1 = 0;
        if (active && (lane <= 30 || A.shift)) {
            if (aks3_phase3(L, up2p, tb_bit, matras, want_c, want_r)) {
                const uint32_t rows_ev = L.rows & ~tb_bit;
                if (want_c) mc = L.brk | rows_ev;
                if (want_r) {
                    mr = L.rchg | rows_ev;
                    t0 = mr & ~(L.PD | L.PO);
                    t1 = mr & ~(L.PD | L.PR);
                }
            } else {
                uint32_t m4[4] = {0u, 0u, 0u, 0u};
                AkSegOut o;
                o.cluster_ends = nullptr; o.cluster_splits = nullptr; o.run_ends = nullptr; o.run_tags = nullptr; o.run_splits = nullptr;
                o.cbase = o.rbase = 0; o.ccap = o.rcap = 0;
                o.lane_masks = m4;
                o.lane_base = cs;
                const int64_t rlo = r_w0 > 0 ? r_w0 - 1 : 0, rhi = r_w2 > B.n_rows ? B.n_rows : r_w2;
                int64_t a, b;
                ak_seg_span(A.T, B.text, B.off, B.n_rows, rlo, lane == 31 ? B.n_rows : rhi, ss, se, A.flags, AK_LOOKBACK_LIMIT, true, o, a, b, st);
                mc = m4[0]; mr = m4[1]; t0 = m4[2]; t1 = m4[3];
            }
        }
        if (lane >= 1 && lane <= 30) { n_c += __popc(mc); n_r += __popc(mr); }
        const int sh = A.shift;
        const uint32_t nc = __shfl_down_sync(0xFFFFFFFFu, mc, 1), nrm = __shfl_down_sync(0xFFFFFFFFu, mr, 1);
        const uint32_t n0 = __shfl_down_sync(0xFFFFFFFFu, t0, 1), n1 = __shfl_down_sync(0xFFFFFFFFu, t1, 1);
        const int64_t w = wt * 30 + (lane - 1);
        if (lane >= 1 && lane <= 30 && w < A.n_words) {
            if (want_c) A.cmask[w] = sh ? __funnelshift_r(mc, nc, sh) : mc;
            if (want_r) {
                A.rmask[w] = sh ? __funnelshift_r(mr, nrm, sh) : mr;
                A.t0[w] = sh ? __funnelshift_r(t0, n0, sh) : t0;
                A.t1[w] = sh ? __funnelshift_r(t1, n1, sh) : t1;
            }
        }
    }
#pragma unroll
    for (int d = 16; d > 0; d >>= 1) {
        n_c += __shfl_xor_sync(0xFFFFFFFFu, n_c, d);
        n_r += __shfl_xor_sync(0xFFFFFFFFu, n_r, d);
    }
    if (lane == 0) {
        if (n_c) atomicAdd((unsigned long long*)&B.result[0], (unsigned long long)n_c);
        if (n_r) atomicAdd((unsigned long long*)&B.result[1], (unsigned long long)n_r);
    }
    ak_raise(B.result, st);
}
```

akshar_b200/csrc/ak_text_core.cuh:

```cuda
#pragma once
#include "ak_unicode.cuh"

#define AK_MAXSEG 256
enum {
    AK_ST_OVERFLOW = 1,
    AK_ST_NFC_SEGMENT = 2,
    AK_ST_PATHOLOGICAL = 4,
    AK_ST_ALPHABET = 8,
    AK_ST_SPIN = 16,
    AK_ST_WORD = 32,
    AK_ST_INTERNAL = 64,
    AK_ST_BAD_ID = 128,
};
#define AK_NORM_ROMAN 1u
#define AK_NORM_FILTER 2u
#define AK_NORM_COLLAPSE 4u
#define AK_NORM_CLEAN 6u
#define AK_NORM_NO_NFC 8u
#define AK_SEG_CLUSTERS 1u
#define AK_SEG_MATRAS 2u
#define AK_SEG_RUNS 4u

AK_HD int64_t ak_row_lower_bound(const int64_t* off, int64_t lo, int64_t hi, int64_t p) {
    while (lo < hi) {
        int64_t mid = (lo + hi) >> 1;
        if (off[mid] >= p) hi = mid; else lo = mid + 1;
    }
    return lo;
}

struct AkNormSink {
    uint8_t* out;
    int64_t cnt;
    int64_t cap;
};
AK_HD void ak_sink_put(AkNormSink& s, uint32_t cp) {
    const int len = ak_utf8_len(cp);
    if (s.out && s.cnt + len <= s.cap) ak_encode(cp, s.out + s.cnt);
    s.cnt += len;
}

struct AkCollapse {
    uint32_t c;
    int n;
    bool pending;
};

AK_HD int ak_post_nfc(const AkTables& T, uint32_t cp, uint32_t props, uint32_t flags, uint32_t* o) {
    int n = 1;
    o[0] = cp;
    if ((flags & AK_NORM_ROMAN) && AK_LATIN_LOWER(props)) {
        o[0] = ak_latin_lower(T, cp);
        if (cp == 0x130u) { o[1] = 0x307u; n = 2; }
        if (flags & AK_NORM_FILTER) props = ak_props(T, o[0]);
    }
    if (flags & AK_NORM_FILTER) {
        int m = 0;
        if (AK_ALLOW(props)) o[m++] = o[0];
        if (n == 2 && AK_ALLOW(ak_props(T, o[1]))) o[m++] = o[1];
        n = m;
    }
    return n;
}

AK_HD void ak_collapse_feed(AkCollapse& st, uint32_t y, AkNormSink& sink) {
    if (y == st.c && y != 0x0Au) {
        if (st.n == 1) { st.n = 2; st.pending = true; }
        else { st.n = 3; st.pending = false; }
    } else {
        if (st.pending) { ak_sink_put(sink, st.c); st.pending = false; }
        ak_sink_put(sink, y);
        st.c = y;
        st.n = 1;
    }
}
AK_HD void ak_collapse_close(AkCollapse& st, uint32_t next, AkNormSink& sink) {
    if (st.pending) {
        if (next != st.c) ak_sink_put(sink, st.c);
        st.pending = false;
    }
}

AK_HD int64_t ak_scan_segment(const AkTables& T, const uint8_t* t, int64_t p, int64_t re, bool& trouble,
                              int64_t scan_limit, uint32_t& status) {
    int len;
    uint32_t cp = ak_decode(t, p, re, len);
    uint32_t w = ak_props(T, cp);
    trouble = AK_QC(w) != 0;
    uint32_t prev_ccc = AK_CCC(w);
    bool after_inert_base = AK_INERT_BASE(w);
    int64_t q = p + len;
    while (q < re) {
        cp = ak_decode(t, q, re, len);
        w = ak_props(T, cp);
        if (AK_NFC_HEAD(w)) break;
        uint32_t cc = AK_CCC(w);
        uint32_t qc = AK_QC(w);
        if (qc == 1u || (qc == 2u && !after_inert_base) || (cc != 0 && prev_ccc > cc)) trouble = true;
        after_inert_base = false;
        prev_ccc = cc;
        q += len;
        if (scan_limit > 0 && q - p > scan_limit) { status |= AK_ST_PATHOLOGICAL; break; }
    }
    return q;
}

AK_HD_NOINLINE int ak_nfc_segment(const AkTables& T, const uint8_t* t, int64_t h, int64_t hend, uint32_t* buf,
                                  uint32_t& status) {
    int n = 0;
    int64_t q = h;
    while (q < hend) {
        int len;
        uint32_t cp = ak_decode(t, q, hend, len);
        if (n + 4 > AK_MAXSEG) { status |= AK_ST_NFC_SEGMENT; break; }
        n = ak_decompose(T, cp, ak_props(T, cp), buf, n);
        q += len;
    }
    return ak_nfc_inplace(T, buf, n);
}

AK_HD int64_t ak_find_head(const AkTables& T, const uint8_t* t, int64_t q, int64_t rs, int64_t re, int64_t limit,
                           uint32_t& status) {
    int64_t q0 = q;
    while (q > rs) {
        int len;
        uint32_t cp = ak_decode(t, q, re, len);
        if (AK_NFC_HEAD(ak_props(T, cp))) break;
        q = ak_prev_start(t, q, rs);
        if (limit > 0 && q0 - q > limit) { status |= AK_ST_PATHOLOGICAL; break; }
    }
    return q;
}

AK_HD_NOINLINE int ak_prev_kept(const AkTables& T, const uint8_t* t, int64_t p, int64_t rs, int64_t re, uint32_t flags,
                                int64_t limit, uint32_t* k, uint32_t& status) {
    int nk = 0;
    int64_t q = p;
    while (nk < 3 && q > rs) {
        if (limit > 0 && p - q > limit) { status |= AK_ST_PATHOLOGICAL; break; }
        int64_t last = ak_prev_start(t, q, rs);
        int64_t h = last;
        bool trouble = false;
        if (!(flags & AK_NORM_NO_NFC)) {
            h = ak_find_head(T, t, last, rs, re, limit, status);
            ak_scan_segment(T, t, h, re, trouble, limit, status);
        }
        if (!trouble) {
            int64_t c = q;
            while (c > h && nk < 3) {
                int64_t cs = ak_prev_start(t, c, rs);
                int len;
                uint32_t cp = ak_decode(t, cs, re, len);
                uint32_t o[2];
                int m = ak_post_nfc(T, cp, ak_props(T, cp), flags, o);
                for (int i = m - 1; i >= 0 && nk < 3; --i) k[nk++] = o[i];
                c = cs;
            }
        } else {
            uint32_t buf[AK_MAXSEG];
            int n = ak_nfc_segment(T, t, h, q, buf, status);
            for (int i = n - 1; i >= 0 && nk < 3; --i) {
                uint32_t o[2];
                int m = ak_post_nfc(T, buf[i], ak_props(T, buf[i]), flags, o);
                for (int j = m - 1; j >= 0 && nk < 3; --j) k[nk++] = o[j];
            }
        }
        q = h;
    }
    return nk;
}

AK_HD_NOINLINE uint32_t ak_next_kept(const AkTables& T, const uint8_t* t, int64_t q, int64_t rs, int64_t re, uint32_t flags,
                                     int64_t limit, uint32_t& status) {
    const int64_t q0 = q;
    while (q < re) {
        if (limit > 0 && q - q0 > limit) { status |= AK_ST_PATHOLOGICAL; break; }
        int len;
        uint32_t cp = ak_decode(t, q, re, len);
        uint32_t w = ak_props(T, cp);
        if (!(flags & AK_NORM_NO_NFC) && (q == rs || AK_NFC_HEAD(w))) {
            bool trouble;
            int64_t hend = ak_scan_segment(T, t, q, re, trouble, limit, status);
            if (trouble) {
                uint32_t buf[AK_MAXSEG];
                int n = ak_nfc_segment(T, t, q, hend, buf, status);
                for (int i = 0; i < n; ++i) {
                    uint32_t o[2];
                    if (ak_post_nfc(T, buf[i], ak_props(T, buf[i]), flags, o) > 0) return o[0];
                }
                q = hend;
                continue;
            }
        }
        uint32_t o[2];
        if (ak_post_nfc(T, cp, w, flags, o) > 0) return o[0];
        q += len;
    }
    return 0xFFFFFFFFu;
}

AK_HD_NOINLINE int64_t ak_norm_span(const AkTables& T, const uint8_t* t, const int64_t* off, int64_t n_rows,
                                    int64_t r_lo, int64_t r_hi, int64_t s, int64_t e, uint32_t flags, int64_t limit,
                                    uint8_t* out, int64_t* out_off, int64_t out_base, uint32_t& status,
                                    int64_t out_cap = 0x7FFFFFFFFFFFFFFFll) {
    const int64_t total_end = off[n_rows];
    const bool clean = (flags & AK_NORM_COLLAPSE) != 0;
    const bool nfc = (flags & AK_NORM_NO_NFC) == 0;
    AkNormSink sink;
    sink.out = out;
    sink.cnt = 0;
    sink.cap = out_cap;
    int64_t p = s;
    if (p < total_end && p > off[0]) {
        const int64_t nr0 = ak_row_lower_bound(off, r_lo, r_hi, p);
        int k = 0;
        while (off[nr0] != s && p < e && p < total_end && p < off[nr0] && k < 3 && (t[p] & 0xC0u) == 0x80u) { ++p; ++k; }
    }
    if (p >= e) return 0;
    int64_t nr = ak_row_lower_bound(off, r_lo, r_hi, p);
    int64_t rs = (off[nr] == p) ? p : off[nr - 1];
    int64_t re = (off[nr] == p) ? p : off[nr];
    AkCollapse st;
    st.c = 0xFFFFFFFFu;
    st.n = 0;
    st.pending = false;
    int64_t inert_until = -1;
    if (p != rs && p < total_end) {
        int len;
        uint32_t cp = ak_decode(t, p, re, len);
        if (nfc && !AK_NFC_HEAD(ak_props(T, cp))) {
            int64_t h = ak_find_head(T, t, p, rs, re, limit, status);
            bool trouble;
            int64_t hend = ak_scan_segment(T, t, h, re, trouble, limit, status);
            if (trouble) p = hend;
            else inert_until = hend;
        }
        if (p >= e) return 0;
        if (clean && p < re) {
            uint32_t k[3];
            int nk = ak_prev_kept(T, t, p, rs, re, flags, limit, k, status);
            if (nk > 0) {
                st.c = k[0];
                st.n = 1;
                if (k[0] != 0x0Au && nk > 1 && k[1] == k[0]) st.n = (nk > 2 && k[2] == k[0]) ? 3 : 2;
            }
        }
        if (p == re) {
            nr = ak_row_lower_bound(off, nr, r_hi, p);
        }
    }
    for (;;) {
        if (p >= e) break;
        while (nr <= n_rows && off[nr] == p) {
            if (out_off) out_off[nr] = out_base + sink.cnt;
            ++nr;
            rs = p;
            st.c = 0xFFFFFFFFu;
            st.n = 0;
            st.pending = false;
            inert_until = -1;
        }
        if (p >= total_end) break;
        re = off[nr];
        int len;
        uint32_t cp = ak_decode(t, p, re, len);
        uint32_t w = ak_props(T, cp);
        bool slow = false;
        int64_t hend = p + len;
        if (nfc && p >= inert_until && (p == rs || AK_NFC_HEAD(w))) {
            bool trouble = AK_QC(w) != 0;
            if (hend < re) {
                int l2;
                uint32_t c2 = ak_decode(t, hend, re, l2);
                if (!AK_NFC_HEAD(ak_props(T, c2))) {
                    int64_t se = ak_scan_segment(T, t, p, re, trouble, limit, status);
                    if (trouble) hend = se; else inert_until = se;
                }
            }
            slow = trouble;
        }
        if (!slow) {
            uint32_t o[2];
            int m = ak_post_nfc(T, cp, w, flags, o);
            for (int i = 0; i < m; ++i) {
                if (clean) ak_collapse_feed(st, o[i], sink); else ak_sink_put(sink, o[i]);
            }
            p += len;
        } else {
            uint32_t buf[AK_MAXSEG];
            int n = ak_nfc_segment(T, t, p, hend, buf, status);
            for (int j = 0; j < n; ++j) {
                uint32_t o[2];
                int m = ak_post_nfc(T, buf[j], ak_props(T, buf[j]), flags, o);
                for (int i = 0; i < m; ++i) {
                    if (clean) ak_collapse_feed(st, o[i], sink); else ak_sink_put(sink, o[i]);
                }
            }
            p = hend;
        }
        if (p >= re) ak_collapse_close(st, 0xFFFFFFFFu, sink);
    }
    if (st.pending) ak_collapse_close(st, ak_next_kept(T, t, p, rs, re, flags, limit, status), sink);
    return sink.cnt;
}

struct AkGState {
    uint8_t prev;
    uint8_t conj;
    uint8_t pict;
    uint8_t ri_odd;
    uint8_t prev_m;
    uint8_t has_prev;
};

AK_HD bool ak_is_matra_or_halant(uint32_t cp) {
    return (cp >= 0x0900u && cp <= 0x0902u) || (cp >= 0x093Eu && cp <= 0x094Du) || (cp >= 0x0951u && cp <= 0x0954u);
}

AK_HD bool ak_g_break(const AkGState& st, uint32_t wb) {
    uint32_t ga = st.prev, gb = AK_GCB(wb);
    if (ga == GCB_CR && gb == GCB_LF) return false;
    if (ga == GCB_CONTROL || ga == GCB_CR || ga == GCB_LF) return true;
    if (gb == GCB_CONTROL || gb == GCB_CR || gb == GCB_LF) return true;
    if (ga == GCB_L && (gb == GCB_L || gb == GCB_V || gb == GCB_LV || gb == GCB_LVT)) return false;
    if ((ga == GCB_LV || ga == GCB_V) && (gb == GCB_V || gb == GCB_T)) return false;
    if ((ga == GCB_LVT || ga == GCB_T) && gb == GCB_T) return false;
    if (gb == GCB_EXTEND || gb == GCB_ZWJ) return false;
    if (gb == GCB_SPACINGMARK) return false;
    if (ga == GCB_PREPEND) return false;
    if (st.conj == 2 && AK_INCB(wb) == INCB_CONSONANT) return false;
    if (st.pict == 2 && AK_EXTPICT(wb)) return false;
    if (ga == GCB_RI && gb == GCB_RI && st.ri_odd) return false;
    return true;
}

AK_HD void ak_g_advance(AkGState& st, uint32_t cp, uint32_t wb) {
    uint32_t gb = AK_GCB(wb), ib = AK_INCB(wb);
    st.ri_odd = (gb == GCB_RI) ? (st.ri_odd ^ 1) : 0;
    if (ib == INCB_CONSONANT) st.conj = 1;
    else if (ib == INCB_LINKER) st.conj = st.conj ? 2 : 0;
    else if (ib != INCB_EXTEND) st.conj = 0;
    if (AK_EXTPICT(wb)) st.pict = 1;
    else if (gb == GCB_EXTEND) st.pict = (st.pict == 1) ? 1 : 0;
    else if (gb == GCB_ZWJ) st.pict = (st.pict == 1) ? 2 : 0;
    else st.pict = 0;
    st.prev = (uint8_t)gb;
    st.prev_m = ak_is_matra_or_halant(cp) ? 1 : 0;
    st.has_prev = 1;
}

AK_HD bool ak_g_sync(uint32_t w) {
    uint32_t g = AK_GCB(w), ib = AK_INCB(w);
    return g != GCB_EXTEND && g != GCB_ZWJ && g != GCB_RI && ib != INCB_LINKER && ib != INCB_EXTEND;
}

struct AkSegOut {
    int32_t* cluster_ends;
    int64_t* cluster_splits;
    int32_t* run_ends;
    uint8_t* run_tags;
    int64_t* run_splits;
    int64_t cbase, rbase;
    int64_t ccap, rcap;
    uint32_t* lane_masks = nullptr;
    int64_t lane_base = 0;
};

AK_HD void ak_seg_put_cluster(const AkSegOut& o, bool write, int64_t cc, int64_t p, int64_t rs) {
    if (!write) return;
    if (o.lane_masks) { o.lane_masks[0] |= 1u << (int)(p - o.lane_base); return; }
    if (o.cbase + cc < o.ccap) o.cluster_ends[o.cbase + cc] = (int32_t)(p - rs);
}
AK_HD void ak_seg_put_run(const AkSegOut& o, bool write, int64_t rc, int64_t p, int64_t rs, uint32_t cur) {
    if (!write) return;
    if (o.lane_masks) {
        const uint32_t b = 1u << (int)(p - o.lane_base);
        o.lane_masks[1] |= b;
        if (cur == (uint32_t)TAG_ROMAN || cur == (uint32_t)TAG_NONE) o.lane_masks[2] |= b;
        if (cur == (uint32_t)TAG_OTHER || cur == (uint32_t)TAG_NONE) o.lane_masks[3] |= b;
        return;
    }
    if (o.rbase + rc < o.rcap) {
        o.run_ends[o.rbase + rc] = (int32_t)(p - rs);
        o.run_tags[o.rbase + rc] = (uint8_t)cur;
    }
}

AK_HD_NOINLINE void ak_seg_span(const AkTables& T, const uint8_t* t, const int64_t* off, int64_t n_rows, int64_t r_lo,
                                int64_t r_hi, int64_t s, int64_t e, uint32_t flags, int64_t limit, bool write,
                                const AkSegOut& o, int64_t& n_clusters, int64_t& n_runs, uint32_t& status) {
    const int64_t total_end = off[n_rows];
    const bool want_c = (flags & AK_SEG_CLUSTERS) != 0, want_r = (flags & AK_SEG_RUNS) != 0;
    const bool matras = (flags & AK_SEG_MATRAS) != 0;
    int64_t cc = 0, rc = 0;
    n_clusters = 0;
    n_runs = 0;
    int64_t p = s;
    if (p < total_end && p > off[0]) {
        const int64_t nr0 = ak_row_lower_bound(off, r_lo, r_hi, p);
        int k = 0;
        while (off[nr0] != s && p < e && p < total_end && p < off[nr0] && k < 3 && (t[p] & 0xC0u) == 0x80u) { ++p; ++k; }
    }
    if (p >= e) return;
    int64_t nr = ak_row_lower_bound(off, r_lo, r_hi, p);
    int64_t rs = (off[nr] == p) ? p : off[nr - 1];
    int64_t re = (off[nr] == p) ? p : off[nr];
    AkGState g;
    g.prev = 0; g.conj = 0; g.pict = 0; g.ri_odd = 0; g.prev_m = 0; g.has_prev = 0;
    uint32_t cur = TAG_NONE;
    int64_t back_lo = rs;
    bool need_cur = p != rs && p < total_end;
    if (p == rs && nr > 0 && off[nr - 1] < p) {
        rs = off[nr - 1];
        back_lo = rs;
        need_cur = true;
    } else if (p != rs && p < total_end) {
        if (want_c) {
            int64_t q = p;
            for (;;) {
                q = ak_prev_start(t, q, rs);
                int len;
                uint32_t cp = ak_decode(t, q, re, len);
                if (ak_g_sync(ak_props(T, cp))) break;
                if (q == rs) break;
                if (limit > 0 && p - q > limit) { status |= AK_ST_PATHOLOGICAL; break; }
            }
            while (q < p) {
                int len;
                uint32_t cp = ak_decode(t, q, re, len);
                ak_g_advance(g, cp, ak_props(T, cp));
                q += len;
            }
        }
    }
    if (want_r && need_cur) {
        int64_t q = p;
        while (q > back_lo) {
            q = ak_prev_start(t, q, back_lo);
            int len;
            uint32_t cp = ak_decode(t, q, p, len);
            uint32_t tg = AK_TAG(ak_props(T, cp));
            if (tg != TAG_DIGIT && tg != TAG_PUNCT) { cur = tg; break; }
            if (limit > 0 && p - q > limit) { status |= AK_ST_PATHOLOGICAL; break; }
        }
    }
    for (;;) {
        if (p >= e) break;
        while (nr <= n_rows && off[nr] == p) {
            if (nr > 0 && p > rs) {
                if (want_c) {
                    ak_seg_put_cluster(o, write, cc, p, rs);
                    ++cc;
                }
                if (want_r) {
                    ak_seg_put_run(o, write, rc, p, rs, cur);
                    ++rc;
                }
            }
            if (write && !o.lane_masks) {
                if (want_c) o.cluster_splits[nr] = o.cbase + cc;
                if (want_r) o.run_splits[nr] = o.rbase + rc;
            }
            ++nr;
            rs = p;
            g.prev = 0; g.conj = 0; g.pict = 0; g.ri_odd = 0; g.prev_m = 0; g.has_prev = 0;
            cur = TAG_NONE;
        }
        if (p >= total_end) break;
        re = off[nr];
        int len;
        uint32_t cp = ak_decode(t, p, re, len);
        uint32_t w = ak_props(T, cp);
        if (want_c) {
            if (g.has_prev) {
                bool brk = ak_g_break(g, w);
                if (matras && (g.prev_m || ak_is_matra_or_halant(cp))) brk = true;
                if (brk) {
                    ak_seg_put_cluster(o, write, cc, p, rs);
                    ++cc;
                }
            }
            ak_g_advance(g, cp, w);
        }
        if (want_r) {
            uint32_t tg = AK_TAG(w);
            if (tg != TAG_DIGIT && tg != TAG_PUNCT) {
                if (cur != TAG_NONE && tg != cur) {
                    ak_seg_put_run(o, write, rc, p, rs, cur);
                    ++rc;
                }
                cur = tg;
            }
        }
        p += len;
    }
    n_clusters = cc;
    n_runs = rc;
}

AK_HD bool ak_final_sigma(const AkTables& T, const uint8_t* t, int64_t p, int len, int64_t rs, int64_t re) {
    int64_t q = p;
    bool before = false;
    while (q > rs) {
        q = ak_prev_start(t, q, rs);
        int l;
        uint32_t w = ak_props(T, ak_decode(t, q, re, l));
        if ((w >> 26) & 1u) continue;
        before = ((w >> 27) & 1u) != 0;
        break;
    }
    if (!before) return false;
    q = p + len;
    while (q < re) {
        int l;
        uint32_t w = ak_props(T, ak_decode(t, q, re, l));
        q += l;
        if ((w >> 26) & 1u) continue;
        return ((w >> 27) & 1u) == 0;
    }
    return true;
}

AK_HD int ak_replace2(uint32_t* a, int n, uint32_t x, uint32_t y, uint32_t r) {
    int m = 0;
    for (int i = 0; i < n;) {
        if (i + 1 < n && a[i] == x && a[i + 1] == y) { a[m++] = r; i += 2; }
        else a[m++] = a[i++];
    }
    return m;
}

AK_HD_NOINLINE int ak_signature_row(const AkTables& T, const uint8_t* t, int64_t rs, int64_t re, uint32_t* a) {
    int n = 0;
    int64_t p = rs;
    uint32_t last = 0xFFFFFFFFu;
    int run = 0;
#define AK_SIG_FEED(c_)                                   \
    do {                                                  \
        uint32_t c = (c_);                                \
        if (c == last) {                                  \
            if (c == 0x0Au) a[n++] = c;                   \
            else if (run < 3) ++run;                      \
        } else {                                          \
            if (run == 2) a[n++] = last;                  \
            a[n++] = c;                                   \
            last = c;                                     \
            run = 1;                                      \
        }                                                 \
    } while (0)
    while (p < re) {
        int len;
        uint32_t cp = ak_decode(t, p, re, len);
        uint32_t w = ak_props(T, cp);
        if (cp == 0x3A3u) AK_SIG_FEED(ak_final_sigma(T, t, p, len, rs, re) ? 0x3C2u : 0x3C3u);
        else if (AK_FULL_LOWER(w) || (cp >= 'A' && cp <= 'Z')) {
            AK_SIG_FEED(ak_full_lower(T, cp));
            if (cp == 0x130u) AK_SIG_FEED(0x307u);
        } else AK_SIG_FEED(cp);
        p += len;
    }
    if (run == 2) a[n++] = last;
#undef AK_SIG_FEED
    for (int pass = 0; pass < 2; ++pass) {
        const uint32_t v = pass == 0 ? 'e' : 'o', r = pass == 0 ? 'i' : 'u';
        if (n >= 2 && a[n - 1] == v && a[n - 2] == v) { a[n - 2] = r; --n; }
        else if (n >= 3 && a[n - 1] == 0x0Au && a[n - 2] == v && a[n - 3] == v) { a[n - 3] = r; a[n - 2] = 0x0Au; --n; }
    }
    n = ak_replace2(a, n, 'a', 'a', 'a');
    n = ak_replace2(a, n, 'k', 'h', 'k');
    n = ak_replace2(a, n, 'g', 'h', 'g');
    n = ak_replace2(a, n, 'c', 'h', 'c');
    n = ak_replace2(a, n, 't', 'h', 't');
    n = ak_replace2(a, n, 'p', 'h', 'p');
    n = ak_replace2(a, n, 'b', 'h', 'b');
    n = ak_replace2(a, n, 'd', 'h', 'd');
    return n;
}
```

akshar_b200/csrc/ak_tok_kernels.cuh:

```cuda
#pragma once

#define AKT_WARP_BYTES 960
#define AKW_THREADS 128
#define AKR_THREADS 256
#define AKL_THREADS 256
#define AKL_PER 4
#define AKL_TILE (AKL_THREADS * AKL_PER)
#define AKT_LONG_ROW 8192

struct AkSlots {
    AkEvent* ev;
    uint32_t* count;
    int cap;
    int shift;
};

__device__ __forceinline__ long long akt_n_wt(const AkBatch& B, int64_t base0) {
    return (B.text_end - base0 + AKT_WARP_BYTES) / AKT_WARP_BYTES;
}

__global__ void ak_cache_guard_kernel(unsigned long long* work, const unsigned long long* image, size_t n_words,
                                      const unsigned long long* inserted, unsigned long long limit, int force) {
    if (!force && *inserted <= limit) return;
    const size_t n2 = n_words / 2;
    const ulonglong2* src = reinterpret_cast<const ulonglong2*>(image);
    ulonglong2* dst = reinterpret_cast<ulonglong2*>(work);
    for (size_t i = (size_t)blockIdx.x * blockDim.x + threadIdx.x; i < n2; i += (size_t)gridDim.x * blockDim.x) dst[i] = src[i];
}
__global__ void ak_cache_guard_reset_kernel(unsigned long long* inserted, unsigned long long limit, int force) {
    if (force || *inserted > limit) *inserted = 0ull;
}

struct AkWordsArgs {
    AkBatch B;
    AkTables T;
    const int64_t* wrow;
    int64_t base0;
    AkSlots S;
    uint8_t* row_flag;
    unsigned int* any_flag;
    uint32_t* row_ev;
    long long* n_wt_out;
    AkBpeDev bpe;
};

template <int KIND>
struct AkScanEnd {
    const AkTables* T;
    const uint8_t* text;
    const int64_t* off;
    int64_t n_rows, cs;
    uint32_t cw;
    __device__ int64_t operator()(int64_t p, int64_t from) const {
        if (KIND == 0) return akb3_scan_end(*T, text, p, from, (cw >> (int)(p - cs)) & 1u, off, n_rows, 0, n_rows);
        const int64_t er = ak_row_lower_bound(off, 0, n_rows, p + 1);
        const int64_t re = off[er];
        int64_t q = from > re ? re : from;
        while (q < re && text[q] != 0x20u) ++q;
        return q;
    }
};

#ifndef AKW_MINB
#define AKW_MINB 8
#endif
template <int KIND>
__global__ void __launch_bounds__(AKW_THREADS, AKW_MINB) ak_words_kernel(const AkWordsArgs A) {
    AkBatch B = A.B;
    if (!ak_batch_begin(B)) return;
    const int lane = threadIdx.x & 31, warp = threadIdx.x >> 5;
    const int64_t tb = B.text_begin, te = B.text_end;
    const long long n_wt = akt_n_wt(B, A.base0);
    if (blockIdx.x == 0 && threadIdx.x == 0) *A.n_wt_out = n_wt;
    uint32_t st = 0;
    for (long long wt = (long long)blockIdx.x * (AKW_THREADS / 32) + warp; wt < n_wt; wt += (long long)gridDim.x * (AKW_THREADS / 32)) {
        const int64_t ws0 = A.base0 + wt * AKT_WARP_BYTES;
        const int64_t cs = ws0 + (int64_t)(lane - 1) * 32;
        const int64_t r_w0 = A.wrow[2 * wt];
        uint32_t x[8];
        uint32_t own;
        {
            int64_t lo = tb - cs, hi = te - cs;
            lo = lo < 0 ? 0 : (lo > 32 ? 32 : lo);
            hi = hi < 0 ? 0 : (hi > 32 ? 32 : hi);
            if (lo == 0 && hi == 32) {
                const uint4 v0 = *reinterpret_cast<const uint4*>(B.text + cs);
                const uint4 v1 = *reinterpret_cast<const uint4*>(B.text + cs + 16);
                x[0] = v0.x; x[1] = v0.y; x[2] = v0.z; x[3] = v0.w;
                x[4] = v1.x; x[5] = v1.y; x[6] = v1.z; x[7] = v1.w;
                own = 0xFFFFFFFFu;
            } else {
                akn3_load_edge(B.text, cs, (int)lo, (int)hi, x);
                own = hi > lo ? ((hi == 32 ? 0xFFFFFFFFu : ((1u << hi) - 1u)) & ~((1u << lo) - 1u)) : 0u;
            }
        }
        int64_t first_row;
        int nrows;
        const uint32_t rows = akn3_lane_rows2(B.off, B.n_rows, r_w0, ws0, lane, first_row, nrows);
        const bool real = lane >= 1 && lane <= 30;
        const int64_t ss = cs < tb ? tb : cs;
        const int64_t se = cs + 32 > te + 1 ? te + 1 : cs + 32;
        const bool active = real && ss < se;
        uint32_t rowsm, wstart, cw, bnd, nb1, nb2;
        if (KIND == 0) {
            AkB3Lane L;
            L.own = own;
            L.rows = rows;
            akb3_phase1(x, L);
            uint32_t dn1n = __shfl_down_sync(0xFFFFFFFFu, L.dn1, 1);
            if (lane == 31) dn1n = 0;
            akb3_phase2(L, dn1n);
            if (L.FOR) akb3_foreign(A.T, B.text, cs, te, L);
            akb3_summary(L);
            const uint32_t up2p = __shfl_up_sync(0xFFFFFFFFu, L.up2, 1);
            akb3_phase3(L, up2p);
            if (active) {
                uint32_t fix = L.UNS & L.own;
                for (uint32_t m = L.LT & L.own; m;) {
                    const int i = akb_ctz(m);
                    m &= m - 1u;
                    if (ak_bpe_special_at(A.bpe, B.text, cs + i, te) >= 0) fix |= 1u << i;
                }
                if (fix) {
                    ake_flag_rows(B.off, B.n_rows, cs, fix, A.row_flag);
                    atomicOr(A.any_flag, 1u);
                }
                if (L.trb) {
                    const int64_t r_lo = r_w0 > 0 ? r_w0 - 1 : 0;
                    if (akb3_changes(A.T, B.text, B.off, B.n_rows, r_lo, L.trb, cs, st)) {
                        ake_flag_rows(B.off, B.n_rows, cs, L.trb, A.row_flag);
                        atomicOr(A.any_flag, 1u);
                    }
                }
            }
            const uint32_t bsend = lane == 31 ? (L.bnd & 0x3FFFFFFFu) : L.bnd;
            nb1 = __shfl_down_sync(0xFFFFFFFFu, bsend, 1);
            nb2 = __shfl_down_sync(0xFFFFFFFFu, bsend, 2);
            if (lane >= 30) nb2 = 0;
            wstart = active ? L.wstart : 0u;
            rowsm = active ? L.rows : 0u;
            cw = L.CW;
            bnd = L.bnd;
        } else {
            AkU3Lane L;
            L.own = own;
            L.rows = rows;
            aku3_phase1(x, L);
            uint32_t upp = __shfl_up_sync(0xFFFFFFFFu, L.up, 1);
            if (lane == 0) upp = 0;
            aku3_phase2(L, upp);
            nb1 = __shfl_down_sync(0xFFFFFFFFu, L.bnd, 1);
            nb2 = __shfl_down_sync(0xFFFFFFFFu, L.bnd, 2);
            if (lane >= 30) nb2 = 0;
            wstart = active ? L.wstart : 0u;
            rowsm = active ? L.rows : 0u;
            cw = 0xFFFFFFFFu;
            bnd = L.bnd;
            if (active && L.exotic) {
                ake_flag_rows(B.off, B.n_rows, cs, L.exotic, A.row_flag);
                atomicOr(A.any_flag, 1u);
            }
        }
        const int n_ev = __popc(rowsm) + __popc(wstart);
        int inc = n_ev;
#pragma unroll
        for (int d = 1; d < 32; d <<= 1) {
            const int y = __shfl_up_sync(0xFFFFFFFFu, inc, d);
            if (lane >= d) inc += y;
        }
        const int total = __shfl_sync(0xFFFFFFFFu, inc, 31);
        const int pre = inc - n_ev;
        if (lane == 0) {
            A.S.count[wt] = (uint32_t)(total < A.S.cap ? total : A.S.cap);
            if (total > A.S.cap) {
                st |= AK_ST_OVERFLOW;
                atomicMax((unsigned long long*)&B.result[3], (unsigned long long)total);
            }
        }
        if (n_ev) {
            const int64_t at = (wt << A.S.shift) + pre;
            const int lane_tail = lane >= 30 ? 62 : lane == 29 ? 94 : 96;
            AkScanEnd<KIND> se;
            se.T = &A.T; se.text = B.text; se.off = B.off; se.n_rows = B.n_rows; se.cs = cs; se.cw = cw;
            ake_lane_events(rowsm, wstart, cw, bnd, nb1, nb2, lane_tail, cs, tb, B.off, B.n_rows, first_row, nrows, at, A.row_ev,
                            A.S.ev + at, (int64_t)A.S.cap - pre, se);
        }
    }
    ak_raise(B.result, st);
}

__global__ void ak_long_rows_kernel(AkBatch B, int64_t limit, uint8_t* row_flag, unsigned int* any_flag) {
    if (!ak_batch_begin(B)) return;
    bool any = false;
    for (int64_t g = (int64_t)blockIdx.x * blockDim.x + threadIdx.x; g < B.n_rows; g += (int64_t)gridDim.x * blockDim.x)
        if (B.off[g + 1] - B.off[g] > limit) { row_flag[g] = 1; any = true; }
    if (any) atomicOr(any_flag, 1u);
}

struct AkRowFixArgs {
    AkBatch B;
    AkRowFixCtx X;
    int64_t base0;
    int cap;
    const uint8_t* row_flag;
    const unsigned int* any_flag;
};

__global__ void __launch_bounds__(128) ak_rowfix_kernel(const AkRowFixArgs A) {
    AkBatch B = A.B;
    if (!ak_batch_begin(B)) return;
    if (*A.any_flag == 0u) return;
    AkRowFixCtx X = A.X;
    X.n_events = (unsigned long long)akt_n_wt(B, A.base0) * (unsigned long long)A.cap;
    X.text = B.text;
    X.off = B.off;
    X.n_rows = B.n_rows;
    X.result = B.result;
    for (int64_t g = (int64_t)blockIdx.x * blockDim.x + threadIdx.x; g < B.n_rows; g += (int64_t)gridDim.x * blockDim.x)
        if (A.row_flag[g]) akr_fix_row(X, g);
}

struct AkResolveArgs {
    AkBatch B;
    AkLookupCtx X;
    int64_t base0;
    AkSlots S;
    unsigned long long* resolved;
    uint32_t* aux;
    int32_t* wt_ids;
    unsigned long long* wt_seg;
    const unsigned int* any_flag;
};

#define AKU_W_KMAX 16
struct AkUniWarpScratch {
    uint32_t cps[AKU_WORD_CPS];
    uint32_t epid[AKU_WORD_CPS][AKU_W_KMAX];
    double best[AKU_WORD_CPS + 1];
    uint32_t bk[AKU_WORD_CPS + 1];
    int n_ids;
    float ratio, wmag;
};

__device__ __forceinline__ double aku_warp_max_d(double v) {
    const uint32_t hi = (uint32_t)__double2hiint(v), lo = (uint32_t)__double2loint(v);
    const uint32_t neg = (uint32_t)((int32_t)hi >> 31);
    const uint32_t khi = hi ^ (neg | 0x80000000u), klo = lo ^ neg;
    const uint32_t H = __reduce_max_sync(0xFFFFFFFFu, khi);
    const uint32_t L = __reduce_max_sync(0xFFFFFFFFu, khi == H ? klo : 0u);
    const uint32_t back = (H & 0x80000000u) ? 0u : 0xFFFFFFFFu;
    return __hiloint2double((int)(H ^ (back | 0x80000000u)), (int)(L ^ back));
}

__device__ __noinline__ bool aku_word_lattice_warp(const AkUniDev& U, const uint8_t* t, int64_t s, uint32_t len, AkUniWarpScratch& S) {
    const int lane = threadIdx.x & 31;
    if (len > 2u * 32u - 8u) return false;
    uint32_t mine = 0;
    uint32_t c[2] = {0u, 0u};
#pragma unroll
    for (int h = 0; h < 2; ++h) {
        const uint32_t q = 2u * (uint32_t)lane + (uint32_t)h;
        if (q < len && (t[s + q] & 0xC0u) != 0x80u) {
            int l;
            c[h] = ak_decode(t, s + q, s + len, l);
            mine |= 1u << h;
        }
    }
    int inc = __popc(mine);
    const int own = inc;
#pragma unroll
    for (int d = 1; d < 32; d <<= 1) {
        const int y = __shfl_up_sync(0xFFFFFFFFu, inc, d);
        if (lane >= d) inc += y;
    }
    const int n = 1 + __shfl_sync(0xFFFFFFFFu, inc, 31);
    if (n > AKU_WORD_CPS) return false;
    {
        int at = 1 + inc - own;
        if (mine & 1u) S.cps[at++] = c[0];
        if (mine & 2u) S.cps[at] = c[1];
        if (lane == 0) S.cps[0] = (U.flags & 4) ? 0x2581u : 0x20u;
    }
    __syncwarp();
    bool deep = false;
    for (int i = lane; i < n; i += 32) {
#pragma unroll
        for (int k = 0; k < AKU_W_KMAX; ++k) S.epid[i][k] = 0u;
        uint32_t node = 0;
        for (int k = 1; i + k <= n; ++k) {
            const unsigned long long v = ak_uni_child(U, node, S.cps[i + k - 1]);
            if (v == AK_EMPTY_KEY) break;
            if (k > AKU_W_KMAX) { deep = true; break; }
            node = (uint32_t)(v >> 32);
            const uint32_t pid1 = (uint32_t)v;
            if (pid1 && U.usable[pid1 - 1u]) S.epid[i][k - 1] = pid1;
        }
    }
    if (__any_sync(0xFFFFFFFFu, deep)) return false;
    if (lane == 0) { S.best[0] = 0.0; S.bk[0] = 0u; }
    __syncwarp();
    double margin = INFINITY, wmag = 0.0;
    for (int j = 1; j <= n; ++j) {
        double cand = -INFINITY;
        uint32_t b = 0u;
        if (lane >= 1 && lane <= AKU_W_KMAX && j - lane >= 0) {
            const int i = j - lane;
            const uint32_t pid1 = S.epid[i][lane - 1];
            const double bi = S.best[i];
            if (pid1 && bi != -INFINITY) {
                cand = bi + (double)U.score[pid1 - 1u];
                b = ((uint32_t)lane << 24) | (pid1 - 1u);
            }
        } else if (lane == 0) {
            const double bi = S.best[j - 1];
            if (bi != -INFINITY && S.epid[j - 1][0] == 0u) {
                cand = bi + (double)U.unk_score;
                b = AK_UNI_UNKBIT | S.cps[j - 1];
            }
        }
        const double a = cand == -INFINITY ? 0.0 : (cand < 0 ? -cand : cand);
        const double m1 = aku_warp_max_d(cand);
        const double wm = aku_warp_max_d(a);
        if (wm > wmag) wmag = wm;
        const unsigned tie = __ballot_sync(0xFFFFFFFFu, cand == m1 && m1 != -INFINITY);
        const int win = tie ? 31 - __clz((int)tie) : 0;
        const double m2 = aku_warp_max_d(lane == win ? -INFINITY : cand);
        const uint32_t wb = __shfl_sync(0xFFFFFFFFu, b, win);
        if (m1 != -INFINITY && m1 - m2 < margin) margin = m1 - m2;
        if (lane == 0) { S.best[j] = m1; S.bk[j] = wb; }
        __syncwarp();
    }
    if (lane == 0) {
        int32_t* ids = reinterpret_cast<int32_t*>(&S.epid[0][0]);
        int cnt = 0;
        for (int j = n; j > 0;) {
            const uint32_t b = S.bk[j];
            if (b & AK_UNI_UNKBIT) { cnt += (U.flags & 8) ? ak_utf8_len(b & 0x1FFFFFu) : 1; j -= 1; }
            else { cnt += 1; j -= (int)((b >> 24) & 0x7Fu); }
        }
        S.n_ids = cnt;
        int at = cnt;
        for (int j = n; j > 0;) {
            const uint32_t b = S.bk[j];
            if (b & AK_UNI_UNKBIT) {
                const uint32_t cp = b & 0x1FFFFFu;
                if (U.flags & 8) {
                    uint8_t enc[4];
                    const int m = ak_encode(cp, enc);
                    for (int q = m - 1; q >= 0; --q) ids[--at] = U.byte_id[enc[q]];
                } else ids[--at] = U.unk_id;
                j -= 1;
            } else {
                ids[--at] = (int32_t)(b & 0xFFFFFFu);
                j -= (int)((b >> 24) & 0x7Fu);
            }
        }
        const double r = margin / (double)n;
        S.ratio = r > 1e30 ? 1e30f : (float)r * 0.999f;
        S.wmag = (float)wmag * 1.001f + 1e-30f;
    }
    __syncwarp();
    return true;
}

#ifndef AKR_MINB0
#define AKR_MINB0 4
#endif
#ifndef AKR_MINB1
#define AKR_MINB1 4
#endif
#ifndef AKE_MINB
#define AKE_MINB 4
#endif
#ifndef AKC_MINB
#define AKC_MINB 8
#endif
template <int KIND>
__global__ void __launch_bounds__(AKR_THREADS, KIND == 0 ? AKR_MINB0 : AKR_MINB1) ak_resolve_kernel(const AkResolveArgs A) {
    AkBatch B = A.B;
    if (!ak_batch_begin(B)) return;
    AkLookupCtx X = A.X;
    X.text = B.text;
    X.off = B.off;
    X.n_rows = B.n_rows;
    X.tb = B.text_begin;
    X.te = B.text_end;
    X.result = B.result;
    X.any_fix = *A.any_flag != 0u ? 1 : 0;
    const int lane = threadIdx.x & 31;
    __shared__ AkUniWarpScratch s_uni[KIND == 1 ? AKR_THREADS / 32 : 1];
    AkUniWarpScratch* const scratch = &s_uni[KIND == 1 ? (threadIdx.x >> 5) : 0];
    const long long n_wt = akt_n_wt(B, A.base0);
    const long long warp0 = ((long long)blockIdx.x * AKR_THREADS + threadIdx.x) >> 5, n_warps = ((long long)gridDim.x * AKR_THREADS) >> 5;
    uint32_t st = 0;
    for (long long wt = warp0; wt < n_wt; wt += n_warps) {
        const int cnt = (int)A.S.count[wt];
        const long long s_wt = wt << A.S.shift;
        int ids = 0;
        unsigned long long seg = 0ull;
        AkEvent ev_next;
        ev_next.pos = 0u;
        ev_next.meta = AKE_DEAD;
        if (lane < cnt) ev_next = A.S.ev[s_wt + lane];
        for (int o = 0; o < cnt; o += 32) {
            const int i = o + lane;
            const AkEvent ev_cur = ev_next;
            if (i + 32 < cnt) ev_next = A.S.ev[s_wt + i + 32];
            unsigned long long r = 0ull;
            uint32_t aux = 0u;
            bool miss = false;
            int64_t miss_p = 0;
            uint32_t miss_len = 0u;
            AkcHit hit;
            hit.slot = hit.free_slot = -1;
            hit.h = hit.want = hit.tag = hit.ids01 = 0ull;
            if (i < cnt) {
                AkEvent ev = ev_cur;
                const uint32_t kind = ev.meta & 7u, len = ev.meta >> 3;
                unsigned long long k[4] = {0ull, 0ull, 0ull, 0ull};
                if (kind <= AKE_WORD && len <= AKC_MAXLEN) akc_key0123(X.text, X.tb + ev.pos, len, X.te, k);
                if (KIND == 1 && kind <= AKE_WORD && len <= 56u && len != AKE_LEN_MAX) {
                    akc_lookup4(X.M.cache, X.text, X.tb + ev.pos, len, k, hit);
                    if (hit.slot >= 0) {
                        const int n = AKC_NTOK(hit.tag);
                        aux = (uint32_t)(hit.tag >> 32);
                        r = n <= 2 ? akr_inline(n, hit.ids01) : akr_cache(n, hit.slot);
                    } else {
                        miss = true;
                        miss_p = X.tb + ev.pos;
                        miss_len = len;
                    }
                } else r = akl_resolve<KIND>(X, ev, k, aux, st);
            }
            if (KIND == 1) {
                for (unsigned mm = __ballot_sync(0xFFFFFFFFu, miss); mm; mm &= mm - 1u) {
                    const int src = __ffs((int)mm) - 1;
                    const int64_t wp = __shfl_sync(0xFFFFFFFFu, miss_p, src);
                    const uint32_t wl = __shfl_sync(0xFFFFFFFFu, miss_len, src);
                    const bool solved = aku_word_lattice_warp(X.M.uni, X.text, wp, wl, *scratch);
                    if (lane == src) {
                        AkMissOut o;
                        if (solved)
                            o = akl_uni_finish(X, wp, wl, hit.free_slot, hit.want, true, true, scratch->n_ids,
                                               reinterpret_cast<const int32_t*>(&scratch->epid[0][0]), scratch->ratio, scratch->wmag);
                        else o = akl_uni_miss(X, wp, wl, hit.free_slot, hit.want, true);
                        st |= o.st;
                        aux = (uint32_t)(akc_aux(o.ratio, o.wmag) >> 32);
                        r = o.slot == -1 ? akr_inline(o.n, o.ids01) : akr_pool(o.n, (unsigned long long)(-3 - o.slot));
                    }
                    __syncwarp();
                }
            }
            if (i < cnt) {
                A.resolved[s_wt + i] = r;
                if (KIND == 1) A.aux[s_wt + i] = aux;
            }
            __syncwarp();
            ids += akr_n(r);
            if (KIND == 1) {
                unsigned long long e = (r >> 62) == AKR_EVENT ? AKS_SEG_FLAG : (unsigned long long)__float_as_uint(aku_aux_wmag(aux));
#pragma unroll
                for (int d = 1; d < 32; d <<= 1) {
                    const unsigned long long y = __shfl_up_sync(0xFFFFFFFFu, e, d);
                    if (lane >= d) e = aks_seg_op(y, e);
                }
                seg = aks_seg_op(seg, __shfl_sync(0xFFFFFFFFu, e, 31));
            }
        }
#pragma unroll
        for (int d = 16; d > 0; d >>= 1) ids += __shfl_xor_sync(0xFFFFFFFFu, ids, d);
        if (lane == 0) {
            A.wt_ids[wt] = ids;
            if (KIND == 1) A.wt_seg[wt] = seg;
        }
    }
    ak_raise(B.result, st);
}

struct AkCheckArgs {
    AkBatch B;
    AkLookupCtx X;
    int64_t base0;
    AkSlots S;
    unsigned long long* resolved;
    const uint32_t* aux;
    const float* wt_seg_before;
    int32_t* wt_ids;
    const unsigned int* any_flag;
};

__global__ void __launch_bounds__(AKL_THREADS, AKC_MINB) ak_unicheck_kernel(const AkCheckArgs A) {
    AkBatch B = A.B;
    if (!ak_batch_begin(B)) return;
    AkLookupCtx X = A.X;
    X.text = B.text;
    X.off = B.off;
    X.n_rows = B.n_rows;
    X.tb = B.text_begin;
    X.te = B.text_end;
    X.result = B.result;
    X.any_fix = *A.any_flag != 0u ? 1 : 0;
    const int lane = threadIdx.x & 31;
    const long long n_wt = akt_n_wt(B, A.base0);
    const long long warp0 = ((long long)blockIdx.x * AKL_THREADS + threadIdx.x) >> 5, n_warps = ((long long)gridDim.x * AKL_THREADS) >> 5;
    for (long long wt = warp0; wt < n_wt; wt += n_warps) {
        const int cnt = (int)A.S.count[wt];
        const long long s_wt = wt << A.S.shift;
        unsigned long long run = (unsigned long long)__float_as_uint(A.wt_seg_before[wt]);
        int delta = 0;
        for (int o4 = 0; o4 < cnt; o4 += 128) {
          uint32_t aux4[4];
          bool row4[4];
#pragma unroll
          for (int q = 0; q < 4; ++q) {
              const int i = o4 + 32 * q + lane;
              aux4[q] = 0u;
              row4[q] = false;
              if (i < cnt) {
                  aux4[q] = A.aux[s_wt + i];
                  row4[q] = (A.resolved[s_wt + i] >> 62) == AKR_EVENT;
              }
          }
#pragma unroll
          for (int q = 0; q < 4; ++q) {
            const int o = o4 + 32 * q;
            if (o >= cnt) break;
            const int i = o + lane;
            const uint32_t aux = aux4[q];
            const bool isrow = row4[q];
            unsigned long long e = isrow ? AKS_SEG_FLAG : (unsigned long long)__float_as_uint(aku_aux_wmag(aux));
#pragma unroll
            for (int d = 1; d < 32; d <<= 1) {
                const unsigned long long y = __shfl_up_sync(0xFFFFFFFFu, e, d);
                if (lane >= d) e = aks_seg_op(y, e);
            }
            const unsigned long long incl = aks_seg_op(run, e);
            run = aks_seg_op(run, __shfl_sync(0xFFFFFFFFu, e, 31));
            if (i < cnt && !isrow && aux != 0u && !aku_robust(aku_aux_ratio(aux), __uint_as_float((uint32_t)incl))) {
                const AkEvent ev = A.S.ev[s_wt + i];
                if ((ev.meta & 7u) <= AKE_WORD) {
                    long long pa;
                    const int n = akl_uni_exact(X, X.tb + ev.pos, ev.meta >> 3, &pa);
                    const unsigned long long r = pa >= 0 ? akr_pool(n, (unsigned long long)pa) : 0ull;
                    delta += akr_n(r) - akr_n(A.resolved[s_wt + i]);
                    A.resolved[s_wt + i] = r;
                }
            }
            __syncwarp();
          }
        }
        if (delta) atomicAdd(&A.wt_ids[wt], delta);
    }
}

struct AkEmitArgs {
    AkBatch B;
    AkLookupCtx X;
    int64_t base0;
    AkSlots S;
    const unsigned long long* resolved;
    const int64_t* wt_base;
    const unsigned int* any_flag;
};

template <class IdT>
__global__ void __launch_bounds__(AKL_THREADS, AKE_MINB) ak_emit_kernel(const AkEmitArgs A) {
    AkBatch B = A.B;
    if (!ak_batch_begin(B)) return;
    AkLookupCtx X = A.X;
    X.text = B.text;
    X.off = B.off;
    X.n_rows = B.n_rows;
    X.tb = B.text_begin;
    X.te = B.text_end;
    X.result = B.result;
    X.any_fix = *A.any_flag != 0u ? 1 : 0;
    IdT* const ids = (IdT*)A.X.ids;
    const int64_t id_cap = A.X.id_cap;
    const int32_t bos = A.X.M.kind == 0 ? A.X.M.bpe.bos : -1, eos = A.X.M.kind == 0 ? A.X.M.bpe.eos : -1;
    const int splits_i32 = A.X.splits_i32;
    const unsigned long long* const cache_e = A.X.M.cache.e;
    const unsigned long long cache_entries = 1ull << A.X.M.cache.bits;
    const int lane = threadIdx.x & 31;
    const long long n_wt = akt_n_wt(B, A.base0);
    const long long warp0 = ((long long)blockIdx.x * AKL_THREADS + threadIdx.x) >> 5, n_warps = ((long long)gridDim.x * AKL_THREADS) >> 5;
    uint32_t st = 0;
    for (long long wt = warp0; wt < n_wt; wt += n_warps) {
        const int cnt = (int)A.S.count[wt];
        const long long s_wt = wt << A.S.shift;
        int64_t at0 = A.wt_base[wt];
        for (int o4 = 0; o4 < cnt; o4 += 128) {
          unsigned long long r4[4];
#pragma unroll
          for (int q = 0; q < 4; ++q) {
              const int i = o4 + 32 * q + lane;
              r4[q] = i < cnt ? A.resolved[s_wt + i] : 0ull;
          }
          const int64_t at_blk = at0;
          int rel4[4] = {0, 0, 0, 0};
          uint32_t later = 0u;
#pragma unroll
          for (int q = 0; q < 4; ++q) {
            const int o = o4 + 32 * q;
            if (o >= cnt) break;
            const unsigned long long r = r4[q];
            const unsigned long long ty = r >> 62;
            const int n = ty == AKR_INLINE ? (int)((r >> 60) & 3ull) : akr_n(r);
            int inc = n;
#pragma unroll
            for (int d = 1; d < 32; d <<= 1) {
                const int y = __shfl_up_sync(0xFFFFFFFFu, inc, d);
                if (lane >= d) inc += y;
            }
            const int64_t at = at0 + (inc - n);
            rel4[q] = (int)(at - at_blk);
            if (ty == AKR_INLINE) {
                if (n > 0) {
                    if (at + n > id_cap) st |= AK_ST_OVERFLOW;
                    else {
                        ids[at] = (IdT)(r & 0x3FFFFFFFull);
                        if (n > 1) ids[at + 1] = (IdT)((r >> 30) & 0x3FFFFFFFull);
                    }
                }
            } else if (o + lane < cnt) later |= 1u << q;
            at0 += __shfl_sync(0xFFFFFFFFu, inc, 31);
          }
          while (later) {
            const int q = __ffs(later) - 1;
            later &= later - 1u;
            const unsigned long long r = q == 0 ? r4[0] : q == 1 ? r4[1] : q == 2 ? r4[2] : r4[3];
            const int64_t at = at_blk + (q == 0 ? rel4[0] : q == 1 ? rel4[1] : q == 2 ? rel4[2] : rel4[3]);
            const int i = o4 + 32 * q + lane;
            const unsigned long long ty = r >> 62;
            const int n = akr_n(r);
            if (ty == AKR_EVENT && !(r & (1ull << 37))) {
                const int64_t g = (int64_t)(r & ((1ull << 37) - 1ull));
                int64_t k2 = at;
                if (at + n > id_cap) st |= AK_ST_OVERFLOW;
                else {
                    if (g > 0 && eos >= 0) ids[k2++] = (IdT)eos;
                    if (splits_i32) ((int32_t*)A.X.splits)[g] = (int32_t)k2;
                    else ((int64_t*)A.X.splits)[g] = k2;
                    if (g < B.n_rows && bos >= 0) ids[k2] = (IdT)bos;
                }
            } else if (ty == AKR_CACHE && (r & 0xFFFFFFFFFFFFFFull) < cache_entries && n <= AKC_MAXTOK) {
                if (at + n > id_cap) st |= AK_ST_OVERFLOW;
                else {
                    const unsigned long long* en = cache_e + (r & 0xFFFFFFFFFFFFFFull) * AKC_ENTRY;
                    unsigned long long v = akc_ld(en + 3);
                    ids[at] = (IdT)(uint32_t)v;
                    ids[at + 1] = (IdT)(uint32_t)(v >> 32);
                    for (int j = 2; j < n; j += 2) {
                        v = akc_ld(en + 8 + (j >> 1));
                        ids[at + j] = (IdT)(uint32_t)v;
                        if (j + 1 < n) ids[at + j + 1] = (IdT)(uint32_t)(v >> 32);
                    }
                }
            } else {
                if (at + n > id_cap) st |= AK_ST_OVERFLOW;
                akl_emit(X, r, A.S.ev + s_wt + i, at);
            }
          }
          __syncwarp();
        }
    }
    ak_raise(B.result, st);
}
```

akshar_b200/csrc/ak_wtok_kernels.cuh:

```cuda
#pragma once
#include "ak_wordtok.cuh"

#define AKWT_THREADS 128

struct AkWtArgs {
    AkBatch B;
    const int64_t* wrow;
    int64_t base0;
    int mode;
    int32_t* count;
    const int64_t* base;
    int32_t* begin;
    int32_t* end;
    int64_t cap;
    int64_t* splits;
    uint8_t* row_flags;
};

template <bool EMIT>
__global__ void __launch_bounds__(AKWT_THREADS, 8) ak_wtok_kernel(const AkWtArgs A) {
    AkBatch B = A.B;
    if (!ak_batch_begin(B)) return;
    const int lane = threadIdx.x & 31, warp = threadIdx.x >> 5;
    const int64_t tb = B.text_begin, te = B.text_end;
    const long long n_wt = akt_n_wt(B, A.base0);
    uint32_t st = 0;
    for (long long wt = (long long)blockIdx.x * (AKWT_THREADS / 32) + warp; wt < n_wt; wt += (long long)gridDim.x * (AKWT_THREADS / 32)) {
        const int64_t ws0 = A.base0 + wt * AKT_WARP_BYTES;
        const int64_t cs = ws0 + (int64_t)(lane - 1) * 32;
        const int64_t r_w0 = A.wrow[2 * wt];
        AkWtLane L;
        uint32_t x[8];
        {
            int64_t lo = tb - cs, hi = te - cs;
            lo = lo < 0 ? 0 : (lo > 32 ? 32 : lo);
            hi = hi < 0 ? 0 : (hi > 32 ? 32 : hi);
            if (lo == 0 && hi == 32) {
                const uint4 v0 = *reinterpret_cast<const uint4*>(B.text + cs);
                const uint4 v1 = *reinterpret_cast<const uint4*>(B.text + cs + 16);
                x[0] = v0.x; x[1] = v0.y; x[2] = v0.z; x[3] = v0.w;
                x[4] = v1.x; x[5] = v1.y; x[6] = v1.z; x[7] = v1.w;
                L.own = 0xFFFFFFFFu;
            } else {
                akn3_load_edge(B.text, cs, (int)lo, (int)hi, x);
                L.own = hi > lo ? ((hi == 32 ? 0xFFFFFFFFu : ((1u << hi) - 1u)) & ~((1u << lo) - 1u)) : 0u;
            }
        }
        L.endbit = (te >= cs && te < cs + 32) ? 1u << (int)(te - cs) : 0u;
        int64_t first_row = 0;
        int nrows = 0;
        if (EMIT) L.rows = akn3_lane_rows2(B.off, B.n_rows, r_w0, ws0, lane, first_row, nrows);
        else L.rows = akn3_lane_rows(B.off, B.n_rows, r_w0, ws0, lane);
        akwt_phase1(x, L);
        uint32_t dnn = __shfl_down_sync(0xFFFFFFFFu, L.dn, 1);
        if (lane == 31) dnn = 0;
        akwt_phase2(L, dnn, A.mode);
        if (L.hl & ~L.DEV) akwt_wide(B.text, cs, te, L);
        akwt_summary(L);
        uint32_t upp = __shfl_up_sync(0xFFFFFFFFu, L.up, 1);
        if (lane == 0) upp = 0;
        const uint32_t open = akwt_phase3(L, upp);
        const bool real = lane >= 1 && lane <= 30;
        const int n_t = real ? __popc(L.T) : 0;
        int inc = n_t | ((real ? nrows : 0) << 16);
#pragma unroll
        for (int d = 1; d < 32; d <<= 1) {
            const int y = __shfl_up_sync(0xFFFFFFFFu, inc, d);
            if (lane >= d) inc += y;
        }
        if (!EMIT) {
            if (lane == 31) A.count[wt] = inc & 0xFFFF;
            continue;
        }
        if (!real) continue;
        const int64_t t_at = A.base[wt] + ((inc & 0xFFFF) - n_t);
        const int64_t e_at = t_at - (int64_t)open;
        const int64_t row_before = r_w0 + ((inc >> 16) - nrows) - 1;
        akwt_emit_lane(L, cs, B.off, B.n_rows, first_row, nrows, row_before, t_at, e_at, A.begin, A.end, A.cap, A.splits, A.row_flags, st);
    }
    ak_raise(B.result, st);
}
```

Before: 120.7.

## Precompute per-lane row-boundary bitmasks in warp-rows kernel for all consumers

The warp-rows kernel now also builds a per-32-byte bitmask of row starts, staged through shared memory, and writes it to a new workspace buffer. The words, wordtok, segment and normalize kernels read one word per lane instead of running a per-warp ballot/shuffle search over the row offsets. Exact first_row/nrows are derived from prefix sums of popcounts, with a fallback to the old search when the counts disagree (for example duplicate offsets from empty rows). This costs extra workspace and a heavier warp-rows pass.

```diff
diff --git a/akshar_b200/csrc/ak_abi_encode.inc b/akshar_b200/csrc/ak_abi_encode.inc
--- a/akshar_b200/csrc/ak_abi_encode.inc
+++ b/akshar_b200/csrc/ak_abi_encode.inc
@@ -58,6 +58,7 @@
     A.bpe = ctx->bpe_d;
     A.base0 = base0;
     A.wrow = (const int64_t*)(base + W.wrow);
+    A.row_bits = (const uint32_t*)(base + W.row_bits);
     A.S = S;
     A.row_flag = (uint8_t*)(base + W.row_flag);
     A.any_flag = any_flag;
@@ -65,7 +66,8 @@
     long long* n_wt_dev = (long long*)(C.ws + 136);
     A.n_wt_out = n_wt_dev;
     const int entries = (int)(n_wt_ub * 2 + 3);
-    ak_warp_rows_kernel<<<(entries + 255) / 256, 256, 0, C.stream>>>(B, base0, entries, (int64_t*)(base + W.wrow));
+    ak_warp_rows_kernel<<<(entries + AK_WARP_ROWS_THREADS - 1) / AK_WARP_ROWS_THREADS, AK_WARP_ROWS_THREADS, 0, C.stream>>>(
+        B, base0, entries, (int64_t*)(base + W.wrow), (uint32_t*)(base + W.row_bits));
     if ((rc = ak_after_launch(ctx, "tok-warp-rows"))) return rc;
     if (kind == 1) {
         ak_long_rows_kernel<<<ctx->sm_count * 4, 256, 0, C.stream>>>(B, AKT_LONG_ROW, A.row_flag, any_flag);
diff --git a/akshar_b200/csrc/ak_abi_text.inc b/akshar_b200/csrc/ak_abi_text.inc
--- a/akshar_b200/csrc/ak_abi_text.inc
+++ b/akshar_b200/csrc/ak_abi_text.inc
@@ -13,10 +13,6 @@
         F.B.n_tiles = (int)((B.text_end - F.base0 + AKF_TILE) / AKF_TILE);
         int64_t* tile_row = (int64_t*)(C.ws + C.L.tile_row);
         F.tile_row = tile_row;
-        const int entries = F.B.n_tiles * AKF_WARPS + 1;
-        ak_warp_rows_kernel<<<(entries + 255) / 256, 256, 0, C.stream>>>(B, F.base0, entries, tile_row);
-        int rc = ak_after_launch(ctx, "warp-rows");
-        if (rc) return rc;
         AkNfWork W;
         const size_t nt = (size_t)F.B.n_tiles;
         char* wp = C.ws + C.L.scratch;
@@ -26,6 +22,14 @@
         W.slow = (AkSlowEntry*)wp;
         W.n_slow = (unsigned int*)(C.ws + 72);
         W.slow_cap = (unsigned int)(nt * AK_BLOCK / 16 + 1024);
+        wp += ak_align((size_t)W.slow_cap * sizeof(AkSlowEntry));
+        uint32_t* row_bits = (uint32_t*)wp;
+        F.row_bits = row_bits;
+        const int entries = F.B.n_tiles * AKF_WARPS + 1;
+        ak_warp_rows_kernel<<<(entries + AK_WARP_ROWS_THREADS - 1) / AK_WARP_ROWS_THREADS, AK_WARP_ROWS_THREADS, 0, C.stream>>>(
+            B, F.base0, entries, tile_row, row_bits);
+        int rc = ak_after_launch(ctx, "warp-rows");
+        if (rc) return rc;
         {
             AkTimed tm(ctx, AKSHAR_TIMER_NORMALIZE_CLASSIFY, C.stream);
             ak_nf3_classify_kernel<<<ak_grid(ctx, ctx->occ_nf3, F.B.n_tiles), AKN3_THREADS, 0, C.stream>>>(F, W);
@@ -101,10 +105,13 @@
     M.t1 = tags ? tags + n_words : nullptr;
     M.n_words = n_words;
     const int64_t n_wt = (B.text_begin + max_bytes - M.base0 + AKN3_WARP_BYTES) / AKN3_WARP_BYTES;
+    const int entries = (int)(n_wt * 2 + 3);
     int64_t* wrow = (int64_t*)(C.ws + C.L.scratch);
+    uint32_t* row_bits = (uint32_t*)(C.ws + C.L.scratch + ak_align((size_t)entries * 8));
     M.wrow = wrow;
-    const int entries = (int)(n_wt * 2 + 3);
-    ak_warp_rows_kernel<<<(entries + 255) / 256, 256, 0, C.stream>>>(B, M.base0, entries, wrow);
+    M.row_bits = row_bits;
+    ak_warp_rows_kernel<<<(entries + AK_WARP_ROWS_THREADS - 1) / AK_WARP_ROWS_THREADS, AK_WARP_ROWS_THREADS, 0, C.stream>>>(
+        B, M.base0, entries, wrow, row_bits);
     if ((rc = ak_after_launch(ctx, "segment-warp-rows"))) return rc;
     {
         AkTimed tm(ctx, AKSHAR_TIMER_SEGMENT, C.stream);
@@ -163,16 +170,19 @@
         const int64_t n_wt = (text_end - F.base0 + AKN3_WARP_BYTES) / AKN3_WARP_BYTES;
         char* wp = C.ws + C.L.scratch;
         int64_t* wrow = (int64_t*)wp;       wp += ak_align(((size_t)n_wt * 2 + 3) * 8);
+        uint32_t* row_bits = (uint32_t*)wp; wp += ak_align(ak_row_bits_bytes((size_t)n_wt * 2 + 3));
         F.c_count = (int32_t*)wp;           wp += ak_align((size_t)n_wt * 4);
         F.r_count = (int32_t*)wp;           wp += ak_align((size_t)n_wt * 4);
         int64_t* c_base = (int64_t*)wp;     wp += ak_align((size_t)n_wt * 8);
         int64_t* r_base = (int64_t*)wp;
         F.wrow = wrow;
+        F.row_bits = row_bits;
         F.c_base = c_base;
         F.r_base = r_base;
         F.o = A.o;
         const int entries = (int)(n_wt * 2 + 3);
-        ak_warp_rows_kernel<<<(entries + 255) / 256, 256, 0, C.stream>>>(C.B, F.base0, entries, wrow);
+        ak_warp_rows_kernel<<<(entries + AK_WARP_ROWS_THREADS - 1) / AK_WARP_ROWS_THREADS, AK_WARP_ROWS_THREADS, 0, C.stream>>>(
+            C.B, F.base0, entries, wrow, row_bits);
         if ((rc = ak_after_launch(ctx, "segment-warp-rows"))) return rc;
         const int grid = ak_grid(ctx, 8, (int)((n_wt + AKSO_THREADS / 32 - 1) / (AKSO_THREADS / 32)));
         ak_seg_off_kernel<false><<<grid, AKSO_THREADS, 0, C.stream>>>(F);
@@ -220,9 +230,11 @@
     const int64_t n_wt = (text_end - A.base0 + AKT_WARP_BYTES) / AKT_WARP_BYTES;
     char* wp = C.ws + C.L.scratch;
     int64_t* wrow = (int64_t*)wp;       wp += ak_align(((size_t)n_wt * 2 + 3) * 8);
+    uint32_t* row_bits = (uint32_t*)wp; wp += ak_align(ak_row_bits_bytes((size_t)n_wt * 2 + 3));
     A.count = (int32_t*)wp;             wp += ak_align((size_t)n_wt * 4);
     int64_t* wt_base = (int64_t*)wp;
     A.wrow = wrow;
+    A.row_bits = row_bits;
     A.base = wt_base;
     A.mode = rule == AKSHAR_WORDS_HINDI ? AKW_MODE_HINDI : AKW_MODE_SPLIT;
     A.begin = d_word_begin;
@@ -231,7 +243,8 @@
     A.splits = d_word_splits;
     A.row_flags = d_row_flags;
     const int entries = (int)(n_wt * 2 + 3);
-    ak_warp_rows_kernel<<<(entries + 255) / 256, 256, 0, C.stream>>>(C.B, A.base0, entries, wrow);
+    ak_warp_rows_kernel<<<(entries + AK_WARP_ROWS_THREADS - 1) / AK_WARP_ROWS_THREADS, AK_WARP_ROWS_THREADS, 0, C.stream>>>(
+        C.B, A.base0, entries, wrow, row_bits);
     if ((rc = ak_after_launch(ctx, "words-warp-rows"))) return rc;
     const int grid = ak_grid(ctx, 8, (int)((n_wt + AKWT_THREADS / 32 - 1) / (AKWT_THREADS / 32)));
     ak_wtok_kernel<false><<<grid, AKWT_THREADS, 0, C.stream>>>(A);
diff --git a/akshar_b200/csrc/ak_common.cuh b/akshar_b200/csrc/ak_common.cuh
--- a/akshar_b200/csrc/ak_common.cuh
+++ b/akshar_b200/csrc/ak_common.cuh
@@ -92,46 +92,36 @@
 
 
 
-__global__ void ak_warp_rows_kernel(AkBatch B, int64_t base0, int n_entries, int64_t* wrow) {
+#define AK_ROW_BITS_PER_ENTRY (AKF_WARP_BYTES / 32)
+#define AK_WARP_ROWS_THREADS 256
+__global__ void __launch_bounds__(AK_WARP_ROWS_THREADS) ak_warp_rows_kernel(AkBatch B, int64_t base0, int n_entries, int64_t* wrow,
+                                                                            uint32_t* row_bits) {
+    __shared__ uint32_t sbits[AK_WARP_ROWS_THREADS * AK_ROW_BITS_PER_ENTRY];
     if (!ak_batch_begin(B)) return;
-    const int k = blockIdx.x * blockDim.x + threadIdx.x;
-    if (k >= n_entries) return;
-    const int64_t pos = base0 + (int64_t)k * AKF_WARP_BYTES;
-    int64_t r = ak_row_lower_bound(B.off, 0, B.n_rows, pos);
-    if (B.off[r] < pos) r = B.n_rows + 1;
-    wrow[k] = r;
+    const int k0 = blockIdx.x * AK_WARP_ROWS_THREADS, k = k0 + threadIdx.x;
+    uint32_t* mine = sbits + threadIdx.x * AK_ROW_BITS_PER_ENTRY;
+    if (k < n_entries) {
+        const int64_t pos = base0 + (int64_t)k * AKF_WARP_BYTES;
+        int64_t r = ak_row_lower_bound(B.off, 0, B.n_rows, pos);
+        if (B.off[r] < pos) r = B.n_rows + 1;
+        wrow[k] = r;
+        ak_row_bits_entry(B.off, B.n_rows, pos, r, AK_ROW_BITS_PER_ENTRY, mine);
+    }
+    __syncthreads();
+    const int n_words = (n_entries - k0 < AK_WARP_ROWS_THREADS ? n_entries - k0 : AK_WARP_ROWS_THREADS) * AK_ROW_BITS_PER_ENTRY;
+    uint32_t* dst = row_bits + (size_t)k0 * AK_ROW_BITS_PER_ENTRY;
+    for (int i = threadIdx.x; i < n_words; i += AK_WARP_ROWS_THREADS) dst[i] = sbits[i];
 }
+
+static inline size_t ak_row_bits_bytes(size_t n_entries) { return n_entries * AK_ROW_BITS_PER_ENTRY * 4; }
 
 
 #define AKN3_THREADS 128
 #define AKN3_WARP_BYTES 960
 
-__device__ __forceinline__ uint32_t akn3_lane_rows(const int64_t* off, int64_t n_rows, int64_t r_w0, int64_t ws, int lane) {
-    uint32_t rows = 0;
-    const int64_t lo = ws - 32, hi = ws + AKN3_WARP_BYTES + 32;
-    for (int64_t r = r_w0;; r += 32) {
-        const int64_t mr = r + lane;
-        const int64_t p = mr <= n_rows ? off[mr] : hi;
-        const unsigned m = __ballot_sync(0xFFFFFFFFu, p < hi);
-        const int cnt = __popc(m);
-        for (int j = 0; j < cnt; ++j) {
-            const int rel = (int)(__shfl_sync(0xFFFFFFFFu, p, j) - lo);
-            if ((rel >> 5) == lane) rows |= 1u << (rel & 31);
-        }
-        if (cnt < 32) break;
-    }
-    for (int64_t r = r_w0 - 1;; r -= 32) {
-        const int64_t mr = r - lane;
-        const int64_t p = mr >= 0 ? off[mr] : lo - 1;
-        const unsigned m = __ballot_sync(0xFFFFFFFFu, p >= lo);
-        const int cnt = __popc(m);
-        for (int j = 0; j < cnt; ++j) {
-            const int rel = (int)(__shfl_sync(0xFFFFFFFFu, p, j) - lo);
-            if ((rel >> 5) == lane) rows |= 1u << (rel & 31);
-        }
-        if (cnt < 32) break;
-    }
-    return rows;
+__device__ __forceinline__ uint32_t ak_lane_row_bits(const uint32_t* row_bits, long long wt, int lane) {
+    const long long j = 30 * wt + lane - 1;
+    return j >= 0 ? row_bits[j] : 0u;
 }
 
 __device__ __forceinline__ uint32_t akn3_lane_rows2(const int64_t* off, int64_t n_rows, int64_t r_w0, int64_t ws, int lane,
diff --git a/akshar_b200/csrc/ak_kernels.cu b/akshar_b200/csrc/ak_kernels.cu
--- a/akshar_b200/csrc/ak_kernels.cu
+++ b/akshar_b200/csrc/ak_kernels.cu
@@ -226,7 +226,7 @@
     return (a > b ? a : b) + 1;
 }
 struct AkTokWs {
-    size_t wrow, count, wt_ids, wt_base, wt_seg, wt_segx, scan_state, row_flag, row_ev, row_fix, pool, longpool, slots, total;
+    size_t wrow, row_bits, count, wt_ids, wt_base, wt_seg, wt_segx, scan_state, row_flag, row_ev, row_fix, pool, longpool, slots, total;
     size_t pool_ints, longpool_ints;
     int64_t n_wt;
 };
@@ -238,6 +238,7 @@
     W.n_wt = n_bytes / AKT_WARP_BYTES + 3;
     size_t at = 0;
     W.wrow = at;       at += ak_align(((size_t)W.n_wt * 2 + 4) * 8);
+    W.row_bits = at;   at += ak_align(ak_row_bits_bytes((size_t)W.n_wt * 2 + 4));
     W.count = at;      at += ak_align((size_t)W.n_wt * 4);
     W.wt_ids = at;     at += ak_align((size_t)W.n_wt * 4);
     W.wt_base = at;    at += ak_align((size_t)W.n_wt * 8);
@@ -270,10 +271,11 @@
     L.scratch = at;
     size_t m = 4 * (size_t)(n_bytes + 2 * n_rows + 2);
     const size_t nf = ak_align(tiles * AK_BLOCK * 4) + ak_align(tiles * AKF_WARPS * 4) + ak_align((tiles * AKF_WARPS + 1) * 8) +
-                      ak_align((tiles * AK_BLOCK / 16 + 1024) * sizeof(AkSlowEntry));
+                      ak_align((tiles * AK_BLOCK / 16 + 1024) * sizeof(AkSlowEntry)) + ak_align(ak_row_bits_bytes(tiles * AKF_WARPS + 2));
     if (nf > m) m = nf;
     const size_t n_wt = (size_t)n_bytes / AKN3_WARP_BYTES + 3;
-    const size_t sg = ak_align((2 * n_wt + 3) * 8) + 2 * ak_align(n_wt * 4) + 2 * ak_align(n_wt * 8);
+    const size_t sg = ak_align((2 * n_wt + 3) * 8) + ak_align(ak_row_bits_bytes(2 * n_wt + 3)) + 2 * ak_align(n_wt * 4) +
+                      2 * ak_align(n_wt * 8);
     if (sg > m) m = sg;
     const size_t tok = ak_tok_ws(n_bytes, n_rows).total;
     if (tok > m) m = tok;
diff --git a/akshar_b200/csrc/ak_norm_kernels.cuh b/akshar_b200/csrc/ak_norm_kernels.cuh
--- a/akshar_b200/csrc/ak_norm_kernels.cuh
+++ b/akshar_b200/csrc/ak_norm_kernels.cuh
@@ -53,6 +53,7 @@
     int64_t out_cap;
     int64_t* out_off;
     const int64_t* tile_row;
+    const uint32_t* row_bits;
     int64_t base0;
     uint32_t flags;
 };
@@ -130,6 +131,7 @@
         const int64_t cs = ws + (int64_t)(lane - 1) * 32;
         AkN3Lane L;
         {
+            L.rows = ak_lane_row_bits(A.row_bits, (long long)tile * (AKF_TILE / AKN3_WARP_BYTES) + warp, lane);
             uint32_t x[8];
             int64_t lo = tb - cs, hi = te - cs;
             lo = lo < 0 ? 0 : (lo > 32 ? 32 : lo);
@@ -144,7 +146,6 @@
                 akn3_load_edge(B.text, cs, (int)lo, (int)hi, x);
                 L.own = hi > lo ? ((hi == 32 ? 0xFFFFFFFFu : ((1u << hi) - 1u)) & ~((1u << lo) - 1u)) : 0u;
             }
-            L.rows = akn3_lane_rows(B.off, B.n_rows, A.tile_row[(size_t)tile * AKF_WARPS + 2 * warp], ws, lane);
             akn3_phase1(x, L);
         }
         uint32_t up1p = __shfl_up_sync(0xFFFFFFFFu, L.up1, 1);
diff --git a/akshar_b200/csrc/ak_seg_kernels.cuh b/akshar_b200/csrc/ak_seg_kernels.cuh
--- a/akshar_b200/csrc/ak_seg_kernels.cuh
+++ b/akshar_b200/csrc/ak_seg_kernels.cuh
@@ -53,6 +53,7 @@
     AkTables T;
     uint32_t flags;
     const int64_t* wrow;
+    const uint32_t* row_bits;
     int64_t base0;
     int32_t* c_count;
     int32_t* r_count;
@@ -78,6 +79,7 @@
         const int64_t cs = ws + (int64_t)(lane - 1) * 32;
         AkS3Lane L;
         {
+            L.rows = ak_lane_row_bits(A.row_bits, wt, lane);
             uint32_t x[8];
             int64_t lo = tb - cs, hi = te - cs;
             lo = lo < 0 ? 0 : (lo > 32 ? 32 : lo);
@@ -92,7 +94,6 @@
                 akn3_load_edge(B.text, cs, (int)lo, (int)hi, x);
                 L.own = hi > lo ? ((hi == 32 ? 0xFFFFFFFFu : ((1u << hi) - 1u)) & ~((1u << lo) - 1u)) : 0u;
             }
-            L.rows = akn3_lane_rows(B.off, B.n_rows, r_w0, ws, lane);
             aks3_phase1(x, L);
         }
         uint32_t dn1n = __shfl_down_sync(0xFFFFFFFFu, L.dn1, 1);
@@ -183,6 +184,7 @@
     AkTables T;
     uint32_t flags;
     const int64_t* wrow;
+    const uint32_t* row_bits;
     int64_t base0;
     uint32_t* cmask;
     uint32_t* rmask;
@@ -208,10 +210,10 @@
     long long n_c = 0, n_r = 0;
     for (long long wt = (long long)blockIdx.x * (AKSM_THREADS / 32) + warp; wt < n_wt; wt += (long long)gridDim.x * (AKSM_THREADS / 32)) {
         const int64_t ws = A.base0 + wt * AKN3_WARP_BYTES;
-        const int64_t r_w0 = A.wrow[2 * wt], r_w2 = A.wrow[2 * wt + 2];
         const int64_t cs = ws + (int64_t)(lane - 1) * 32;
         AkS3Lane L;
         {
+            L.rows = ak_lane_row_bits(A.row_bits, wt, lane);
             uint32_t x[8];
             int64_t lo = tb - cs, hi = te - cs;
             lo = lo < 0 ? 0 : (lo > 32 ? 32 : lo);
@@ -226,7 +228,6 @@
                 akn3_load_edge(B.text, cs, (int)lo, (int)hi, x);
                 L.own = hi > lo ? ((hi == 32 ? 0xFFFFFFFFu : ((1u << hi) - 1u)) & ~((1u << lo) - 1u)) : 0u;
             }
-            L.rows = akn3_lane_rows(B.off, B.n_rows, r_w0, ws, lane);
             aks3_phase1(x, L);
         }
         uint32_t dn1n = __shfl_down_sync(0xFFFFFFFFu, L.dn1, 1);
@@ -256,6 +257,7 @@
                 o.cbase = o.rbase = 0; o.ccap = o.rcap = 0;
                 o.lane_masks = m4;
                 o.lane_base = cs;
+                const int64_t r_w0 = A.wrow[2 * wt], r_w2 = A.wrow[2 * wt + 2];
                 const int64_t rlo = r_w0 > 0 ? r_w0 - 1 : 0, rhi = r_w2 > B.n_rows ? B.n_rows : r_w2;
                 int64_t a, b;
                 ak_seg_span(A.T, B.text, B.off, B.n_rows, rlo, lane == 31 ? B.n_rows : rhi, ss, se, A.flags, AK_LOOKBACK_LIMIT, true, o, a, b, st);
diff --git a/akshar_b200/csrc/ak_text_core.cuh b/akshar_b200/csrc/ak_text_core.cuh
--- a/akshar_b200/csrc/ak_text_core.cuh
+++ b/akshar_b200/csrc/ak_text_core.cuh
@@ -27,6 +27,37 @@
         if (off[mid] >= p) hi = mid; else lo = mid + 1;
     }
     return lo;
+}
+
+AK_HD void ak_row_bits_entry(const int64_t* off, int64_t n_rows, int64_t pos, int64_t r, int n_words, uint32_t* bits) {
+    const int64_t end = pos + 32 * (int64_t)n_words;
+    int w = 0;
+    uint32_t m = 0;
+    bool more = true;
+    while (more && r <= n_rows) {
+        int64_t q[8];
+#pragma unroll
+        for (int i = 0; i < 8; ++i) q[i] = r + i <= n_rows ? off[r + i] : end;
+#pragma unroll
+        for (int i = 0; i < 8; ++i) {
+            if (q[i] >= end) {
+                more = false;
+                break;
+            }
+            const int j = (int)((q[i] - pos) >> 5);
+            for (; w < j; ++w) {
+                bits[w] = m;
+                m = 0;
+            }
+            m |= 1u << (int)((q[i] - pos) & 31);
+        }
+        r += 8;
+        if (more && q[0] == q[7] && r <= n_rows) r = ak_row_lower_bound(off, r, n_rows, q[7] + 1);
+    }
+    for (; w < n_words; ++w) {
+        bits[w] = m;
+        m = 0;
+    }
 }
 
 struct AkNormSink {
diff --git a/akshar_b200/csrc/ak_tok_kernels.cuh b/akshar_b200/csrc/ak_tok_kernels.cuh
--- a/akshar_b200/csrc/ak_tok_kernels.cuh
+++ b/akshar_b200/csrc/ak_tok_kernels.cuh
@@ -35,6 +35,7 @@
     AkBatch B;
     AkTables T;
     const int64_t* wrow;
+    const uint32_t* row_bits;
     int64_t base0;
     AkSlots S;
     uint8_t* row_flag;
@@ -76,7 +77,7 @@
     for (long long wt = (long long)blockIdx.x * (AKW_THREADS / 32) + warp; wt < n_wt; wt += (long long)gridDim.x * (AKW_THREADS / 32)) {
         const int64_t ws0 = A.base0 + wt * AKT_WARP_BYTES;
         const int64_t cs = ws0 + (int64_t)(lane - 1) * 32;
-        const int64_t r_w0 = A.wrow[2 * wt];
+        const uint32_t rows = ak_lane_row_bits(A.row_bits, wt, lane);
         uint32_t x[8];
         uint32_t own;
         {
@@ -94,9 +95,6 @@
                 own = hi > lo ? ((hi == 32 ? 0xFFFFFFFFu : ((1u << hi) - 1u)) & ~((1u << lo) - 1u)) : 0u;
             }
         }
-        int64_t first_row;
-        int nrows;
-        const uint32_t rows = akn3_lane_rows2(B.off, B.n_rows, r_w0, ws0, lane, first_row, nrows);
         const bool real = lane >= 1 && lane <= 30;
         const int64_t ss = cs < tb ? tb : cs;
         const int64_t se = cs + 32 > te + 1 ? te + 1 : cs + 32;
@@ -126,6 +124,7 @@
                     atomicOr(A.any_flag, 1u);
                 }
                 if (L.trb) {
+                    const int64_t r_w0 = A.wrow[2 * wt];
                     const int64_t r_lo = r_w0 > 0 ? r_w0 - 1 : 0;
                     if (akb3_changes(A.T, B.text, B.off, B.n_rows, r_lo, L.trb, cs, st)) {
                         ake_flag_rows(B.off, B.n_rows, cs, L.trb, A.row_flag);
@@ -161,15 +160,21 @@
                 atomicOr(A.any_flag, 1u);
             }
         }
-        const int n_ev = __popc(rowsm) + __popc(wstart);
-        int inc = n_ev;
+        const int64_t r_w0 = A.wrow[2 * wt], r_w2 = A.wrow[2 * wt + 2];
+        int nrows = __popc(rowsm);
+        const int n_ev = nrows + __popc(wstart);
+        const int mine = n_ev | (nrows << 16);
+        int inc = mine;
 #pragma unroll
         for (int d = 1; d < 32; d <<= 1) {
             const int y = __shfl_up_sync(0xFFFFFFFFu, inc, d);
             if (lane >= d) inc += y;
         }
-        const int total = __shfl_sync(0xFFFFFFFFu, inc, 31);
-        const int pre = inc - n_ev;
+        const int all = __shfl_sync(0xFFFFFFFFu, inc, 31);
+        const int total = all & 0xFFFF;
+        const int pre = (inc - mine) & 0xFFFF;
+        int64_t first_row = r_w0 + ((inc - mine) >> 16);
+        if (r_w2 - r_w0 != (all >> 16)) akn3_lane_rows2(B.off, B.n_rows, r_w0, ws0, lane, first_row, nrows);
         if (lane == 0) {
             A.S.count[wt] = (uint32_t)(total < A.S.cap ? total : A.S.cap);
             if (total > A.S.cap) {
diff --git a/akshar_b200/csrc/ak_wtok_kernels.cuh b/akshar_b200/csrc/ak_wtok_kernels.cuh
--- a/akshar_b200/csrc/ak_wtok_kernels.cuh
+++ b/akshar_b200/csrc/ak_wtok_kernels.cuh
@@ -6,6 +6,7 @@
 struct AkWtArgs {
     AkBatch B;
     const int64_t* wrow;
+    const uint32_t* row_bits;
     int64_t base0;
     int mode;
     int32_t* count;
@@ -28,8 +29,8 @@
     for (long long wt = (long long)blockIdx.x * (AKWT_THREADS / 32) + warp; wt < n_wt; wt += (long long)gridDim.x * (AKWT_THREADS / 32)) {
         const int64_t ws0 = A.base0 + wt * AKT_WARP_BYTES;
         const int64_t cs = ws0 + (int64_t)(lane - 1) * 32;
-        const int64_t r_w0 = A.wrow[2 * wt];
         AkWtLane L;
+        L.rows = ak_lane_row_bits(A.row_bits, wt, lane);
         uint32_t x[8];
         {
             int64_t lo = tb - cs, hi = te - cs;
@@ -47,10 +48,6 @@
             }
         }
         L.endbit = (te >= cs && te < cs + 32) ? 1u << (int)(te - cs) : 0u;
-        int64_t first_row = 0;
-        int nrows = 0;
-        if (EMIT) L.rows = akn3_lane_rows2(B.off, B.n_rows, r_w0, ws0, lane, first_row, nrows);
-        else L.rows = akn3_lane_rows(B.off, B.n_rows, r_w0, ws0, lane);
         akwt_phase1(x, L);
         uint32_t dnn = __shfl_down_sync(0xFFFFFFFFu, L.dn, 1);
         if (lane == 31) dnn = 0;
@@ -62,7 +59,8 @@
         const uint32_t open = akwt_phase3(L, upp);
         const bool real = lane >= 1 && lane <= 30;
         const int n_t = real ? __popc(L.T) : 0;
-        int inc = n_t | ((real ? nrows : 0) << 16);
+        int nrows = real ? __popc(L.rows) : 0;
+        int inc = n_t | (nrows << 16);
 #pragma unroll
         for (int d = 1; d < 32; d <<= 1) {
             const int y = __shfl_up_sync(0xFFFFFFFFu, inc, d);
@@ -72,10 +70,24 @@
             if (lane == 31) A.count[wt] = inc & 0xFFFF;
             continue;
         }
+        const int64_t r_w0 = A.wrow[2 * wt];
+        int rows_before = (inc >> 16) - nrows;
+        int64_t first_row = r_w0 + rows_before;
+        if (A.wrow[2 * wt + 2] - r_w0 != (__shfl_sync(0xFFFFFFFFu, inc, 31) >> 16)) {
+            akn3_lane_rows2(B.off, B.n_rows, r_w0, ws0, lane, first_row, nrows);
+            if (!real) nrows = 0;
+            rows_before = nrows;
+#pragma unroll
+            for (int d = 1; d < 32; d <<= 1) {
+                const int y = __shfl_up_sync(0xFFFFFFFFu, rows_before, d);
+                if (lane >= d) rows_before += y;
+            }
+            rows_before -= nrows;
+        }
         if (!real) continue;
         const int64_t t_at = A.base[wt] + ((inc & 0xFFFF) - n_t);
         const int64_t e_at = t_at - (int64_t)open;
-        const int64_t row_before = r_w0 + ((inc >> 16) - nrows) - 1;
+        const int64_t row_before = r_w0 + rows_before - 1;
         akwt_emit_lane(L, cs, B.off, B.n_rows, first_row, nrows, row_before, t_at, e_at, A.begin, A.end, A.cap, A.splits, A.row_flags, st);
     }
     ak_raise(B.result, st);
```

After: 126.6 (median of 6 runs). 1.05x the previous value.
